# dalek-cryptography/zkp

Hardware: AMD Instinct MI355X
Metric: proofs/sec + batch-verifies/sec, CMZ13 10-attr credential, 1/2/4/8 MI355X (higher is better)
Workload: dtype u32x9 (29-bit limbs, u64 accumulate)

## Files before the change

### include/zkp_mi355x.h

```cpp
#ifndef ZKP_MI355X_H
#define ZKP_MI355X_H

#include <stddef.h>
#include <stdint.h>

#ifdef __cplusplus
extern "C" {
#endif

#define ZKP_OK 0
#define ZKP_ERR_HIP (-1)
#define ZKP_ERR_ARG (-2)
#define ZKP_ERR_NO_DEVICE (-3)
#define ZKP_ERR_OOM (-4)

#define ZKP_VARTIME 0
#define ZKP_CT 1

typedef struct zkp_ctx zkp_ctx;

int zkp_ctx_create(zkp_ctx** out, int device_id);
void zkp_ctx_destroy(zkp_ctx* ctx);
int zkp_ctx_set_stream(zkp_ctx* ctx, void* hip_stream);
int zkp_ctx_synchronize(zkp_ctx* ctx);
// ... 158 lines not shown
                  uint8_t* out );
int zkp_sc_muladd_dev(zkp_ctx* ctx, uint64_t n, const uint8_t* d_a, uint32_t a_stride, const uint8_t* d_b, uint32_t b_stride, const uint8_t* d_c,
                      uint32_t c_stride, uint8_t* d_out );
int zkp_sc_random(zkp_ctx* ctx, uint64_t n, const uint8_t key[32], uint64_t nonce, uint8_t* out );
int zkp_sc_random_dev(zkp_ctx* ctx, uint64_t n, const uint8_t key[32], uint64_t nonce, uint8_t* d_out );
int zkp_sc_hash_from_bytes_sha512(zkp_ctx* ctx, uint64_t n, const uint8_t* msgs, const uint64_t* offsets , uint8_t* out );
int zkp_sc_hash_from_bytes_sha512_dev(zkp_ctx* ctx, uint64_t n, const uint8_t* d_msgs, uint64_t msgs_len, const uint64_t* d_offsets ,
                                      uint8_t* d_out );

int zkp_transcripts_append_message(zkp_ctx* ctx, uint32_t N, int shared_initial, uint8_t* ts , const char* label,
                                   const uint8_t* msgs, const uint64_t* offsets );
int zkp_transcripts_append_message_dev(zkp_ctx* ctx, uint32_t N, int shared_initial, const uint8_t* d_ts_in, uint8_t* d_ts_out,
                                       const char* label, const uint8_t* d_msgs, uint64_t msgs_len, const uint64_t* d_offsets );
int zkp_transcripts_challenge_bytes(zkp_ctx* ctx, uint32_t N, uint8_t* ts , const char* label, uint32_t len,
                                    uint8_t* out );
int zkp_transcripts_challenge_bytes_dev(zkp_ctx* ctx, uint32_t N, uint8_t* d_ts , const char* label, uint32_t len,
                                        uint8_t* d_out );
uint32_t zkp_strobe_pos_after_append(uint32_t strobe_pos, uint64_t label_len, uint64_t msg_len);

int zkp_mul_base(zkp_ctx* ctx, uint64_t n, const uint8_t* scalars , uint8_t* out );
int zkp_mul_base_dev(zkp_ctx* ctx, uint64_t n, const uint8_t* d_scalars , uint8_t* d_out );
int zkp_mul_points(zkp_ctx* ctx, uint64_t n, const uint8_t* scalars, uint32_t s_stride, const uint8_t* points, uint32_t p_stride, int flags,
                   uint8_t* out , uint8_t* status );
int zkp_mul_points_dev(zkp_ctx* ctx, uint64_t n, const uint8_t* d_scalars, uint32_t s_stride, const uint8_t* d_points, uint32_t p_stride, int flags,
                       uint8_t* d_out , uint8_t* d_status );

#define ZKP_PT_ADD 0
#define ZKP_PT_SUB 1
int zkp_add_points(zkp_ctx* ctx, uint64_t n, const uint8_t* a, uint32_t a_stride, const uint8_t* b, uint32_t b_stride, int op,
                   uint8_t* out , uint8_t* status );
int zkp_add_points_dev(zkp_ctx* ctx, uint64_t n, const uint8_t* d_a, uint32_t a_stride, const uint8_t* d_b, uint32_t b_stride, int op,
                       uint8_t* d_out , uint8_t* d_status );
int zkp_sum_points(zkp_ctx* ctx, uint32_t n_sums, const uint32_t* off , const uint32_t* pidx ,
                   const uint8_t* neg , const uint8_t* points , uint32_t n_points,
                   uint8_t* out , uint8_t* status );
int zkp_sum_points_dev(zkp_ctx* ctx, uint32_t n_sums, const uint32_t* d_off , const uint32_t* d_pidx ,
                       const uint8_t* d_neg , const uint8_t* d_points , uint32_t n_points, uint32_t n_terms,
                       uint8_t* d_out , uint8_t* d_status );
uint32_t zkp_sum_points_group(void);

#define ZKP_DLOG_FOUND 0
#define ZKP_DLOG_INVALID 1
#define ZKP_DLOG_NOT_FOUND 2
int zkp_ctx_prepare_dlog(zkp_ctx* ctx, uint32_t baby_bits);
uint32_t zkp_dlog_baby_bits(zkp_ctx* ctx);
int zkp_dlog_base(zkp_ctx* ctx, uint64_t n, const uint8_t* points , uint32_t bits, uint64_t* out , uint8_t* status );
int zkp_dlog_base_dev(zkp_ctx* ctx, uint64_t n, const uint8_t* d_points , uint32_t bits, uint64_t* d_out , uint8_t* d_status );
uint32_t zkp_dlog_group(void);
uint32_t zkp_dlog_chunk(void);
uint32_t zkp_dlog_slice_chunks(uint64_t n);

int zkp_msm_segments(zkp_ctx* ctx, uint32_t n_msm, const uint32_t* off , const uint8_t* scalars ,
                     const uint32_t* pidx , const uint8_t* points , uint32_t n_points, int flags,
                     uint8_t* out , uint8_t* status );
int zkp_msm_segments_dev(zkp_ctx* ctx, uint32_t n_msm, const uint32_t* d_off , const uint8_t* d_scalars ,
                         const uint32_t* d_pidx , const uint8_t* d_points , uint32_t n_points,
                         uint32_t n_terms, int flags, uint8_t* d_out , uint8_t* d_status );

enum {
  ZKP_K_DECODE = 0,
  ZKP_K_TERMS = 1,
  ZKP_K_REDUCE = 2,
  ZKP_K_SORT = 3,
  ZKP_K_BUCKET = 4,
  ZKP_K_COMBINE = 5,
  ZKP_K_TRANSCRIPT = 6,
  ZKP_K_SCALARS = 7,
  ZKP_K_TABLES = 8,
  ZKP_K_COUNT = 9
};
int zkp_ctx_last_timing(zkp_ctx* ctx, float* kernel_ms , float* total_ms);
int zkp_ctx_last_kernels(zkp_ctx* ctx, int kind, char* buf, size_t cap);
int zkp_ctx_set_profiling(zkp_ctx* ctx, int enabled);

#ifdef ZKP_BUILD_TEST_HOOKS
int zkp_debug_quad_selftest(zkp_ctx* ctx, uint32_t n, const uint8_t* pairs , uint8_t* out );
int zkp_debug_row_selftest(zkp_ctx* ctx, uint32_t n, const uint8_t* pairs , uint8_t* out );
int zkp_debug_wave_cycles(zkp_ctx* ctx, uint64_t* out, uint32_t cap);
int zkp_debug_sha512(zkp_ctx* ctx, uint64_t n, const uint8_t* msgs, const uint64_t* offsets , uint8_t* out );
int zkp_debug_last_schedule(zkp_ctx* ctx, char* buf, size_t cap);
int zkp_debug_ragged_blocks(const uint8_t* transcripts, uint32_t N, uint32_t* idx, uint32_t* blocks, uint32_t cap);
int zkp_debug_fill_workspace(zkp_ctx* ctx, size_t min_bytes, uint32_t word);
size_t zkp_debug_ws_bytes(zkp_ctx* ctx);
enum { ZKP_TESTOPT_DUMMY_LAUNCHES = 1001, ZKP_TESTOPT_GENERIC_CLASSIFIER = 1002, ZKP_TESTOPT_WAVE_CYCLES = 1003, ZKP_TESTOPT_PIP_MERGE = 1004, ZKP_TESTOPT_VOUCH_REDUCED = 1005 };
#endif

#ifdef __cplusplus
}
#endif
#endif
```

### zkp_amd/csrc/fused_flows.h

```cpp
#pragma once
#include "merlin_prog.h"
#include "transcript_kernels.h"

namespace zkp {

__global__ void __launch_bounds__(256)
k_wide_reduce(uint32_t n, const uint8_t* __restrict__ wide, uint8_t* __restrict__ out) {
  const uint32_t i = blockIdx.x * blockDim.x + threadIdx.x;
  if (i >= n) return;
  sc lo, hi, r;
  load_vec<2>(lo.v, wide + 64 * (size_t)i);
  load_vec<2>(hi.v, wide + 64 * (size_t)i + 32);
  sc_from_wide(r, lo, hi);
  store_vec<2>(out + 32 * (size_t)i, r.v);
}

__global__ void __launch_bounds__(256)
k_neg_reduce(uint32_t n, const uint8_t* in, uint8_t* out) {
  const uint32_t i = blockIdx.x * blockDim.x + threadIdx.x;
  if (i >= n) return;
  sc a, r;
  load_vec<2>(a.v, in + 32 * (size_t)i);
  sc_reduce(r, a);
  sc_neg(r, r);
// ... 1091 lines not shown
  if (o.end + terms_path_ws(n_points, N * T1, N * nc, tk) > ws_bound)
    return fail(ZKP_ERR_ARG, "internal: verify_core's term path does not fit the workspace its caller sized");
  const ws_view w{static_cast<char*>(c->ws)};
  tr_bufs hb{};
  hb.src[SRC_TABLE] = d_tbl; hb.src[SRC_COMS] = w.u8(o.coms);
  hb.dst[DST_CHAL] = w.u8(o.wchal);
  HIP_TRY(hipMemsetAsync(w.base + o.failed, 0, (size_t)N * 4, c->stream));
  prof_begin(c);
  const size_t lanes = std::max<size_t>((size_t)N * T1, (size_t)N * nc) + 1;
  tk.throughput = throughput;
  if (pl.d_order) { tk.map.N = N; tk.map.nc = nc; tk.map.order = pl.d_order; }
  tk.stmt.off = w.u32(o.off); tk.stmt.pidx = w.u32(o.pidx);
  uint64_t* d_img = pl.img_bytes ? reinterpret_cast<uint64_t*>(w.base + o.img) : nullptr;
  offer_program(c, pl.a, N, hb, d_ts, nullptr, w.u32(o.failed), throughput, overlap, d_img);
  {
    hipStream_t main;
    int rc = side_begin(c, &main, overlap);
    if (rc) { c->pending_tr.offered = c->pending_tr.active = false; return rc; }
    if (late_inputs && late_early) {
      hipStream_t cur = c->stream;
      c->stream = main;
      rc = (*late_inputs)();
      c->stream = cur;
      late_inputs = nullptr;
      if (rc) { (void)side_end(c, main, overlap); c->pending_tr.offered = c->pending_tr.active = false; return rc; }
    }
    if (!stmt_classify_applies(tk, N * T1))
      hipLaunchKernelGGL(k_stmt_index, grid1(lanes, 256), dim3(256), 0, c->stream, N, T1, nc, pl.s.ns, pl.d_tarr, pl.d_tarr + nc + 1 + T1, w.u32(o.off), w.u32(o.pidx));
    rc = msm_terms_path(c, N * nc, w.u32(o.off), nullptr, w.u32(o.pidx), d_tbl, n_points, N * T1, ZKP_VARTIME, w.u8(o.coms), w.u8(o.st8), nullptr, o.end, true, PH_POINTS, tk);
    const int rc2 = side_end(c, main, overlap);
    if (rc || rc2) { c->pending_tr.offered = c->pending_tr.active = false; return rc ? rc : rc2; }
  }
  if (late_inputs) { const int rc = (*late_inputs)(); if (rc) return rc; }
  run_program_pending(c, pl.a, N, hb, d_ts, nullptr, w.u32(o.failed), throughput, d_img);
  prof_mark(c, ZKP_K_TRANSCRIPT);
  hipLaunchKernelGGL(k_neg_reduce, grid1(N, 256), dim3(256), 0, c->stream, N, d_claim, w.u8(o.mc));
  if (T1) hipLaunchKernelGGL(k_stmt_scalars, grid1((size_t)N * T1, 256), dim3(256), 0, c->stream, N, T1, m, pl.d_tarr + nc + 1, d_resp, w.u8(o.mc), w.u8(o.sc), 0u);
  prof_mark(c, ZKP_K_SCALARS);
  HIP_TRY(hipGetLastError());
  int rc = side_join(c, overlap);
  if (rc) return rc;
  rc = msm_terms_path(c, N * nc, w.u32(o.off), w.u8(o.sc), w.u32(o.pidx), d_tbl, n_points, N * T1, ZKP_VARTIME, w.u8(o.coms), w.u8(o.st8), nullptr, o.end, true, PH_SCALARS, tk);
  if (rc) return rc;
  run_program(c, pl.b, N, hb, d_ts, nullptr, w.u32(o.failed), throughput, d_img);
  prof_mark(c, ZKP_K_TRANSCRIPT);
  hipLaunchKernelGGL(k_wide_reduce, grid1(N, 256), dim3(256), 0, c->stream, N, w.u8(o.wchal), w.u8(o.chal));
  hipLaunchKernelGGL(k_verify_finish, grid1(N, 256), dim3(256), 0, c->stream, N, nc, pl.s.ns, m, w.u8(o.chal), d_claim, d_resp, w.u8(o.st8), w.u32(o.failed),
                     reinterpret_cast<const dev_affine*>(w.base + o.end), pl.d_tarr + nc + 1 + 2 * (size_t)T1, (uint32_t)pl.s.unref.size(), d_results);
  prof_mark(c, ZKP_K_SCALARS);
  HIP_TRY(hipGetLastError());
  return ZKP_OK;
}

struct batch_inter { size_t sc, failed, flags, wchal, mc, part, img, end; };
batch_inter batch_carve(const fused_plan& pl, size_t start, uint32_t K = 1) {
  const size_t N = pl.N, ns = pl.s.ns, N_each = N / (K ? K : 1), total = (size_t)K * ns + ((size_t)pl.s.ni + pl.s.nc) * N, nblk = (size_t)K * ((N_each + 255) / 256);
  carve cv;
  cv.off = start;
  batch_inter o;
  o.sc = cv.take(total * 32 + 32);
  o.failed = cv.take(N * 4 + 4);
  o.flags = cv.take((size_t)K * 4);
  o.wchal = cv.take(N * 64 + 64);
  o.mc = cv.take(N * 32 + 32);
  o.part = cv.take((ns ? ns : 1) * (nblk ? nblk : 1) * 32);
  o.img = cv.take(pl.img_bytes);
  o.end = cv.off;
  return o;
}
size_t optional_many_ws(uint64_t n_each, uint32_t K) {
  switch (pick_c(n_each)) {
    case 7: return pip_ws<7>(n_each, K);
    case 10: return pip_ws<10>(n_each, K);
    case 11: return pip_ws<11>(n_each, K);
    default: return pip_ws<16>(n_each, K);
  }
}
int batch_core(zkp_ctx* c, const fused_plan& pl, const batch_inter& o, uint8_t* d_ts, uint8_t* d_pts, const uint8_t* d_coms,
               const uint8_t* d_resp, const uint8_t* d_w, uint8_t* d_out ,
               uint32_t* d_status , bool throughput, uint32_t K = 1,
               bool overlap = false, const std::function<int()>* late_ts = nullptr, const std::function<int()>* late_scalars = nullptr, bool late_early = false) {
  const uint32_t N = pl.N, nc = pl.s.nc, ns = pl.s.ns, ni = pl.s.ni, N_each = N / K;
  const size_t n_each = (size_t)ns + ((size_t)ni + nc) * N_each;
  const ws_view w{static_cast<char*>(c->ws)};
  uint32_t* shared = nullptr;
  if (K > 1) {
    shared = w.u32(o.flags);
    HIP_TRY(hipMemsetAsync(shared, 0, (size_t)K * 4, c->stream));
  } else if (N && n_each > kSmallOptional && pl.a.n) {
    shared = w.u32(o.failed) + N;
  }
  if (!shared) HIP_TRY(hipMemsetAsync(d_status, 0, 8, c->stream));
  prof_begin(c);
  ZKP_SCHED(c, STATUS_SHARED, shared != nullptr);
  uint64_t* d_img = pl.img_bytes ? reinterpret_cast<uint64_t*>(w.base + o.img) : nullptr;
  const bool split = overlap && K == 1 && N && shared && transcript_steps(c, pl.a, N, throughput, d_img);
  if (N) {
    tr_bufs hb{};
    hb.src[SRC_TABLE] = d_pts; hb.src[SRC_COMS] = d_coms;
    hb.dst[DST_CHAL] = w.u8(o.wchal);
    if (split) {
      run_program(c, pl.a, N, hb, d_ts, nullptr, w.u32(o.failed), throughput, d_img, true, 1);
      hipStream_t main;
      int rc = side_begin(c, &main, true);
      if (rc) return rc;
      if (late_early) {
        hipStream_t cur = c->stream;
        c->stream = main;
        if (late_ts) rc = (*late_ts)();
        if (!rc && late_scalars) rc = (*late_scalars)();
        c->stream = cur;
        late_ts = late_scalars = nullptr;
        if (rc) { (void)side_end(c, main, true); return rc; }
      }
      if (nc) hipLaunchKernelGGL(k_transpose_commitments, grid1((size_t)N * nc, 256), dim3(256), 0, c->stream, N, nc, d_coms, d_pts + 32 * ((size_t)ns + (size_t)ni * N));
      rc = msm_optional_impl(c, n_each, w.u8(o.sc), d_pts, d_out, d_status, o.end, shared, 1);
      const int rc2 = side_end(c, main, true);
      if (rc || rc2) return rc ? rc : rc2;
      if (late_ts) { rc = (*late_ts)(); if (rc) return rc; }
      run_program(c, pl.a, N, hb, d_ts, nullptr, w.u32(o.failed), throughput, d_img, true, 2);
    } else {
      if (late_ts) { const int rc = (*late_ts)(); if (rc) return rc; }
      run_program(c, pl.a, N, hb, d_ts, nullptr, w.u32(o.failed), throughput, d_img, true);
    }
    prof_mark(c, ZKP_K_TRANSCRIPT);
    if (late_scalars) { const int rc = (*late_scalars)(); if (rc) return rc; }
    const size_t lanes = std::max<size_t>(std::max<size_t>(N, (size_t)N * nc), (size_t)N * pl.s.m);
    hipLaunchKernelGGL(k_batch_after_transcript, grid1(lanes, 256), dim3(256), 0, c->stream, N, N_each, nc, pl.s.m, w.u32(o.failed),
                       shared ? shared : d_status + 1, 1u, shared ? 2u : 1u, w.u8(o.wchal), w.u8(o.mc), split ? (const uint8_t*)nullptr : d_coms,
                       d_pts + 32 * ((size_t)ns + (size_t)ni * N), d_resp);
  }
  launch_coeff_build(c, pl.s, N_each, pl.d_inc, w.u8(o.mc), d_resp, d_w, w.u8(o.sc), w.u32(o.part), K);
  prof_mark(c, ZKP_K_SCALARS);
  HIP_TRY(hipGetLastError());
  if (split) {
    const int rc = side_join(c, true);
    if (rc) return rc;
    return msm_optional_impl(c, n_each, w.u8(o.sc), d_pts, d_out, d_status, o.end, shared, 2);
  }
  if (K == 1) return msm_optional_impl(c, n_each, w.u8(o.sc), d_pts, d_out, d_status, o.end, shared);
  pip_seg seg;
  seg.K = K; seg.ns = ns; seg.N_each = N_each;
  switch (pick_c(n_each)) {
    case 7: return pip_run<7>(c, (uint32_t)n_each, w.u8(o.sc), d_pts, d_out, d_status, o.end, shared, seg);
    case 10: return pip_run<10>(c, (uint32_t)n_each, w.u8(o.sc), d_pts, d_out, d_status, o.end, shared, seg);
    case 11: return pip_run<11>(c, (uint32_t)n_each, w.u8(o.sc), d_pts, d_out, d_status, o.end, shared, seg);
    default: return pip_run<16>(c, (uint32_t)n_each, w.u8(o.sc), d_pts, d_out, d_status, o.end, shared, seg);
  }
}

struct each_inter { size_t failed, wchal, mc, off, sc, pidx, out, st8, img, end; };
each_inter each_carve(const fused_plan& pl, size_t start) {
  const size_t N = pl.N, K = (size_t)pl.s.np + pl.s.nc;
  carve cv;
  cv.off = start;
  each_inter o;
  o.failed = cv.take(N * 4 + 4);
  o.wchal = cv.take(N * 64 + 64);
  o.mc = cv.take(N * 32 + 32);
  o.off = cv.take((N + 1) * 4);
  o.sc = cv.take(N * K * 32 + 32);
  o.pidx = cv.take(N * K * 4 + 4);
  o.out = cv.take(N * 32 + 32);
  o.st8 = cv.take(N + 4);
  o.img = cv.take(pl.img_bytes);
  o.end = cv.off;
  return o;
}
terms_cfg each_terms_cfg(const fused_plan& pl) {
  terms_cfg k;
  k.max_tables = pl.N >= 2 ? pl.s.ns : 0;
  k.max_ladder = (uint32_t)std::min<uint64_t>(((uint64_t)pl.s.ni + pl.s.nc) * pl.N + pl.s.ns, 0xffffffffu);
  k.teeth = pl.N >= 6 ? 16 : 4;
  return k;
}
struct straus_inter { size_t pts, tab, digits, spart, end; };
constexpr uint32_t kStrausMaxLanes = 8, kStrausMaxOpsPerLane = 60;
constexpr uint32_t kStrausWinParts = 32, kStrausWinMaxProofs = 65536;
inline uint32_t straus_win_parts(const zkp_ctx* c, const fused_plan& pl) {
  const uint32_t K = pl.s.np + pl.s.nc, N = pl.N;
  if (K > 64 || c->each_straus_lanes) return 0;
  if (c->each_straus_wins) return c->each_straus_wins;
  return N < kStrausWinMaxProofs ? kStrausWinParts : 0;
}
inline uint32_t straus_lanes(const zkp_ctx* c, const fused_plan& pl) {
  const uint32_t K = pl.s.np + pl.s.nc, N = pl.N;
  uint32_t L = c->each_straus_lanes ? std::min<uint32_t>(c->each_straus_lanes, kStrausMaxLanes) : (N >= 65536 ? 1u : (N >= 32768 ? 2u : (N >= 16384 ? 4u : 8u)));
  while (L < kStrausMaxLanes && (K + L - 1) / L > kStrausMaxOpsPerLane) L *= 2;
  return std::max(1u, std::min(std::min(L, kStrausMaxLanes), K));
}
inline bool each_uses_straus(const zkp_ctx* c, const fused_plan& pl) {
  const uint64_t K = (uint64_t)pl.s.np + pl.s.nc;
  return c->each_straus && K >= 4 && (K + kStrausMaxLanes - 1) / kStrausMaxLanes <= kStrausMaxOpsPerLane;
}
straus_inter straus_carve(const zkp_ctx* c, const fused_plan& pl, size_t start) {
  const size_t N = pl.N, K = (size_t)pl.s.np + pl.s.nc, n_points = (size_t)pl.s.ns + (size_t)pl.s.ni * N + N * pl.s.nc;
  carve cv;
  cv.off = start;
  straus_inter o;
  o.pts = cv.take(n_points * sizeof(dev_affine));
  o.tab = cv.take(n_points * 8 * sizeof(straus_entry) + 128);
  o.digits = cv.take(N * K * 9 * 4);
  o.spart = cv.take(N * (std::max(kStrausMaxLanes, straus_win_parts(c, pl)) + 1) * sizeof(dev_ext));
  o.end = cv.off;
  return o;
}
int each_core(zkp_ctx* c, const fused_plan& pl, const each_inter& o, uint8_t* d_ts, const uint8_t* d_tbl, const uint8_t* d_resp,
              const uint8_t* d_w, uint8_t* d_results, bool overlap) {
  const uint32_t N = pl.N, nc = pl.s.nc, ns = pl.s.ns, ni = pl.s.ni, K = pl.s.np + nc;
  const uint32_t n_points = ns + ni * N + N * nc;
  const ws_view w{static_cast<char*>(c->ws)};
  const uint8_t* d_coms = d_tbl + 32 * ((size_t)ns + (size_t)ni * N);
  tr_bufs hb{};
  hb.src[SRC_TABLE] = d_tbl; hb.src[SRC_COMS] = d_coms;
  hb.dst[DST_CHAL] = w.u8(o.wchal);
  HIP_TRY(hipMemsetAsync(w.base + o.failed, 0, (size_t)N * 4, c->stream));
  prof_begin(c);
  const bool straus = each_uses_straus(c, pl);
  straus_inter so{};
  dev_affine* pts = nullptr;
  straus_entry* tab = nullptr;
  if (straus) {
    so = straus_carve(c, pl, o.end);
    if (so.end > c->ws_bytes) return fail(ZKP_ERR_ARG, "internal: workspace too small");
// ... 292 lines not shown
```

### zkp_amd/csrc/zkp_kernels.hip

```cpp
#include <hip/hip_runtime.h>
#include <sys/syscall.h>
#include <unistd.h>
#include <cctype>
#include <cstdio>
#include <cstring>
#include <algorithm>
#include <atomic>
#include <functional>
#include <map>
#include <memory>
#include <mutex>
#include <set>
#include <string>
#include <vector>
#include "../../include/zkp_mi355x.h"
#include "dev_layout.h"

using namespace zkp;

__device__ __forceinline__ uint32_t sel8(const uint32_t w[8], int j) {
  uint32_t r = w[0];
#pragma unroll
  for (int i = 1; i < 8; ++i) r = (j == i) ? w[i] : r;
  return r;
}

#include "sc25519.h"
#include "hot_tables.h"
#include "quad.h"
#include "rowfe.h"
#include "comb_tables.h"
#include "point_mul.h"
#include "point_sum.h"
#include "dlog.h"
#include "transcript_kernels.h"
#include "sha512.h"

__global__ void __launch_bounds__(256, 2)
k_decode_affine(uint32_t n, const uint8_t* __restrict__ enc, dev_affine* __restrict__ out, const uint32_t* __restrict__ only) {
  const uint32_t i = blockIdx.x * blockDim.x + threadIdx.x;
  if (i >= n) return;
  if (only && !only[i]) { out[i].valid = 1; return; }
  uint32_t w[8];
  load_vec<2>(w, enc + 32 * (size_t)i);
  ge_p3 p;
  const uint32_t ok = ristretto_decode(p, w);
  store_affine(out + i, p, ok);
}

__device__ __forceinline__ void term_generic(uint32_t t, const uint8_t* __restrict__ scalars, const uint32_t* __restrict__ pidx,
                                             uint32_t n_points, const dev_affine* __restrict__ pts, dev_ext* __restrict__ partial) {
  uint32_t s[8], e[8], top;
  load_vec<2>(s, scalars + 32 * (size_t)t);
  sc_add_pattern(e, top, s, 0xAAAAAAAAu);
  ge_p3 P, P2, acc;
  const uint32_t pi = pidx[t];
  load_affine(P, pts + (pi < n_points ? pi : 0u));
  ge_cached c1, c2;
  ge_to_cached(c1, P);
  ge_double<true>(P2, P);
  ge_to_cached(c2, P2);
  ge_identity(acc);
  fe_cmov(acc.X, P.X, top);
  fe_cmov(acc.Y, P.Y, top);
  fe_cmov(acc.T, P.T, top);
#pragma unroll 1
  for (int j = 7; j >= 0; --j) {
    uint32_t cur = sel8(e, j);
#pragma unroll 1
    for (int k = 0; k < 16; ++k) {
      const uint32_t d = cur >> 30;
      cur <<= 2;
      ge_double<false>(acc, acc);
      ge_double<true>(acc, acc);
      const uint32_t neg = (uint32_t)(d < 2);
      const uint32_t mag = neg ? 2u - d : d - 2u;
      ge_cached sel;
      ge_cached_identity(sel);
      ge_cached_cmov(sel, c1, (uint32_t)(mag == 1));
      ge_cached_cmov(sel, c2, (uint32_t)(mag == 2));
      ge_cached_cneg(sel, neg);
      ge_add_cached(acc, acc, sel);
    }
  }
  store_ext(partial + t, acc);
}

__global__ void __launch_bounds__(256, 2)
k_terms_r4(uint32_t n_terms, const uint8_t* __restrict__ scalars, const uint32_t* __restrict__ pidx,
           uint32_t n_points, const dev_affine* __restrict__ pts, dev_ext* __restrict__ partial) {
  const uint32_t t = blockIdx.x * blockDim.x + threadIdx.x;
  if (t < n_terms) term_generic(t, scalars, pidx, n_points, pts, partial);
}

#ifdef ZKP_BUILD_TEST_HOOKS
__device__ uint64_t* g_wave_cycles = nullptr;
__device__ uint32_t g_wave_cycles_cap = 0;
#define ZKP_WAVE_T0 const uint64_t wave_t0_ = __builtin_readcyclecounter();
#define ZKP_WAVE_T1(cls) do { const uint64_t dt_ = __builtin_readcyclecounter() - wave_t0_; const uint32_t wi_ = blockIdx.x * 4 + (threadIdx.x >> 6); \
  if (g_wave_cycles && (threadIdx.x & 63u) == 0 && wi_ < g_wave_cycles_cap) g_wave_cycles[wi_] = ((uint64_t)(cls) << 56) | (dt_ & 0x00ffffffffffffffull); } while (0)
#else
#define ZKP_WAVE_T0
#define ZKP_WAVE_T1(cls)
#endif

enum : int { LOOKUP_XBAR = 0, LOOKUP_SCAN = 1, LOOKUP_LDS = 2 };
template <int LOOKUP>
constexpr int terms_lds_uint4() {
  if (LOOKUP == LOOKUP_XBAR) return XBAR_LDS_UINT4 > 512 ? XBAR_LDS_UINT4 : 512;
  return HOT_ROW_CHUNKS * HOT_COPIES > GROUP_LDS_UINT4 ? HOT_ROW_CHUNKS * HOT_COPIES : GROUP_LDS_UINT4;
// ... 276 lines not shown
  if (i < n_msm) {
    ge_p3 acc;
    const uint32_t g = msm_of_lane(map, i);
    const uint32_t bad = msm_sum(acc, g, off, pidx, n_points, pts, partial);
    status[g] = (STATUS_T)bad;
    ristretto_dc_state s;
    ristretto_dc_prepare(s, x, acc);
    const uint32_t zero = fe_iszero(x);
    zflag[i] = (uint8_t)zero;
    if (zero) fe_1(x);
    uint32_t* st = states + (size_t)i * 54;
#pragma unroll
    for (int k = 0; k < 9; ++k) {
      st[k] = s.e.v[k]; st[9 + k] = s.f.v[k]; st[18 + k] = s.g.v[k]; st[27 + k] = s.h.v[k]; st[36 + k] = s.eg.v[k]; st[45 + k] = s.fh.v[k];
      xs[(size_t)i * 9 + k] = x.v[k];
    }
  }
  tree_put(tree, ENC_BLOCK + tid, x);
  __syncthreads();
  tree_up(tree, tid);
  if (tid < 9) bprod[(size_t)blockIdx.x * 9 + tid] = tree.node[1][tid];
}

__global__ void __launch_bounds__(ENC_BLOCK)
k_encode_invert(uint32_t n_blocks, const uint32_t* __restrict__ bprod, uint32_t* __restrict__ binv) {
  __shared__ enc_tree tree;
  encode_invert_block(tree, threadIdx.x, blockIdx.x * ENC_BLOCK + threadIdx.x, n_blocks, bprod, binv);
}

__global__ void __launch_bounds__(ENC_BLOCK, 2)
k_encode_finish(uint32_t n_msm, const uint32_t* __restrict__ off, const uint32_t* __restrict__ pidx, uint32_t n_points,
                const dev_affine* __restrict__ pts, const dev_ext* __restrict__ partial, const uint32_t* __restrict__ states,
                const uint32_t* __restrict__ xs, const uint32_t* __restrict__ binv, const uint8_t* __restrict__ zflag,
                const uint8_t* __restrict__ status8, const uint32_t* __restrict__ status32, uint8_t* __restrict__ out, const msm_map map) {
  __shared__ enc_tree tree;
  const int tid = threadIdx.x;
  const uint32_t i = blockIdx.x * ENC_BLOCK + tid;
  fe x;
  fe_1(x);
  if (i < n_msm) {
#pragma unroll
    for (int k = 0; k < 9; ++k) x.v[k] = xs[(size_t)i * 9 + k];
    FE_TRACK(fe_set_ub_tight(x));
  }
  tree_put(tree, ENC_BLOCK + tid, x);
  __syncthreads();
  tree_up(tree, tid);
  if (tid < 9) tree.node[1][tid] = binv[(size_t)blockIdx.x * 9 + tid];
  __syncthreads();
  tree_down(tree, tid);
  if (i >= n_msm) return;
  const uint32_t g = msm_of_lane(map, i);
  uint32_t w[8];
  if (zflag[i]) {
    ge_p3 acc;
    msm_sum(acc, g, off, pidx, n_points, pts, partial);
    ge_double<true>(acc, acc);
    ristretto_encode(w, acc);
  } else {
    ristretto_dc_state s;
    const uint32_t* st = states + (size_t)i * 54;
#pragma unroll
    for (int k = 0; k < 9; ++k) {
      s.e.v[k] = st[k]; s.f.v[k] = st[9 + k]; s.g.v[k] = st[18 + k]; s.h.v[k] = st[27 + k]; s.eg.v[k] = st[36 + k]; s.fh.v[k] = st[45 + k];
    }
    fe inv;
    tree_get(inv, tree, ENC_BLOCK + tid);
    ristretto_dc_finish(w, s, inv);
  }
  const uint32_t bad = status8 ? (uint32_t)status8[g] : status32[g];
  if (bad) {
#pragma unroll
    for (int k = 0; k < 8; ++k) w[k] = 0;
  }
  store_vec<2>(out + 32 * (size_t)g, w);
}

__global__ void k_iota_single_msm(uint32_t n, uint32_t* __restrict__ pidx, uint32_t* __restrict__ off) {
  const uint32_t i = blockIdx.x * blockDim.x + threadIdx.x;
  if (i < n) pidx[i] = i;
  if (i == 0) { off[0] = 0; off[1] = n; }
}

template <int C>
struct pip_cfg {
  static constexpr int W = (256 + C - 1) / C;
  static constexpr int W1 = W + 1;
  static constexpr uint32_t B = 1u << (C - 1);
  static constexpr uint32_t B1 = B + 1;
  static constexpr uint32_t kword(int j) {
    uint32_t r = 0;
    for (int w = 0; w < W; ++w) {
      const int bit = C - 1 + C * w;
      if (bit / 32 == j) r |= 1u << (bit % 32);
    }
    return r;
  }
};

struct pip_seg {
  uint32_t K = 1, ns = 0, N_each = 0;
};
__device__ __forceinline__ void pip_seg_src(const pip_seg& seg, uint32_t b, uint32_t l, size_t& si, size_t& pi) {
  si = pi = l;
  if (seg.K > 1) {
    if (l < seg.ns) {
      si = (size_t)b * seg.ns + l;
    } else {
      const uint32_t q = l - seg.ns, r = q / seg.N_each, j = q - r * seg.N_each;
      const size_t col = ((size_t)r * seg.K + b) * seg.N_each + j;
      si = (size_t)seg.K * seg.ns + col;
      pi = (size_t)seg.ns + col;
    }
  }
}

template <int C, int PHASE = 3>
__global__ void __launch_bounds__(256, 2)
k_pip_prepare(uint32_t n, const pip_seg seg, const uint8_t* __restrict__ scalars, const uint8_t* __restrict__ points,
              dev_niels* __restrict__ niels, uint32_t* __restrict__ digits, uint32_t* __restrict__ invalid) {
  using cfg = pip_cfg<C>;
  const uint32_t i = blockIdx.x * blockDim.x + threadIdx.x, b = blockIdx.y;
  if (i >= n) return;
  size_t si, pi;
  pip_seg_src(seg, b, i, si, pi);
  niels += (size_t)b * n;
  digits += (size_t)b * cfg::W1 * n;
  if constexpr (PHASE & 1) {
    uint32_t w[8];
    load_vec<2>(w, points + 32 * pi);
    ge_p3 p;
    const uint32_t ok = ristretto_decode(p, w);
    ge_niels q;
    ge_affine_to_niels(q, p);
    store_niels(niels + i, q, ok);
    if (!ok) atomicOr(invalid + b, 1u);
  }
  if constexpr (!(PHASE & 2)) return;
  uint32_t s[8], e[10];
  load_vec<2>(s, scalars + 32 * si);
  const uint32_t flip = sc_fold_sign(s);
  {
    uint64_t c = 0;
#pragma unroll
    for (int j = 0; j < 9; ++j) {
      c += (uint64_t)(j < 8 ? s[j] : 0u) + cfg::kword(j);
      e[j] = (uint32_t)c;
      c >>= 32;
    }
    e[9] = 0;
  }
#pragma unroll
  for (int w = 0; w < cfg::W1; ++w) {
    const int pos = C * w, lo = pos >> 5, sh = pos & 31;
    uint32_t v = e[lo] >> sh;
    if (sh + C > 32) v |= e[lo + 1] << (32 - sh);
    v &= (1u << C) - 1u;
    uint32_t mag, neg;
    if (w < cfg::W) {
      neg = (uint32_t)(v < cfg::B);
      mag = neg ? cfg::B - v : v - cfg::B;
    } else {
      neg = 0;
      mag = v;
    }
    digits[(size_t)w * n + i] = mag | ((neg ^ flip) << 31);
  }
}

__device__ __forceinline__ uint32_t part_len(uint32_t cnt, uint32_t L) {
  const uint32_t r = (uint32_t)ceilf(sqrtf((float)cnt));
  return r > 4 * L ? 4 * L : (r > L ? r : L);
}
__device__ __forceinline__ uint32_t part_count(uint32_t cnt, uint32_t L) {
  const uint32_t pl = part_len(cnt, L);
  return (cnt + pl - 1) / pl;
}

__global__ void __launch_bounds__(256)
k_pip_scan(uint32_t bins, uint32_t L, const uint32_t* __restrict__ hist, uint32_t* __restrict__ start,
           uint32_t* __restrict__ cursor, uint32_t* __restrict__ vstart) {
  __shared__ uint32_t part[256];
  __shared__ uint32_t vpart[256];
  const uint32_t w = blockIdx.x, tid = threadIdx.x;
  const uint32_t chunk = (bins + 255) / 256;
  const uint32_t lo = min(tid * chunk, bins), hi = min(lo + chunk, bins);
  const uint32_t* h = hist + (size_t)w * bins;
  uint32_t sum = 0, vsum = 0;
  for (uint32_t b = lo; b < hi; ++b) { sum += h[b]; vsum += part_count(h[b], L); }
  part[tid] = sum;
  vpart[tid] = vsum;
  __syncthreads();
  for (uint32_t d = 1; d < 256; d <<= 1) {
    const uint32_t v = tid >= d ? part[tid - d] : 0;
    const uint32_t vv = tid >= d ? vpart[tid - d] : 0;
    __syncthreads();
    part[tid] += v;
    vpart[tid] += vv;
    __syncthreads();
  }
  uint32_t run = part[tid] - sum, vrun = vpart[tid] - vsum;
  for (uint32_t b = lo; b < hi; ++b) {
    start[(size_t)w * bins + b] = run;
    cursor[(size_t)w * bins + b] = run;
    vstart[(size_t)w * (bins + 1) + b] = vrun;
    run += h[b];
    vrun += part_count(h[b], L);
  }
  if (tid == 255) vstart[(size_t)w * (bins + 1) + bins] = vpart[255];
}

template <int C>
struct sort_cfg {
  static constexpr int THREADS = C >= 16 ? 1024 : 256;
  static constexpr uint32_t TILE = C >= 16 ? 65536u : 2048u;
};

template <int C>
__global__ void __launch_bounds__(sort_cfg<C>::THREADS)
k_pip_tile_hist(uint32_t n, const uint32_t* __restrict__ digits, uint32_t* __restrict__ tilehist) {
  using cfg = pip_cfg<C>;
  __shared__ uint32_t h[cfg::B1];
  const uint32_t w = blockIdx.y, t = blockIdx.x, tiles = gridDim.x;
  for (uint32_t b = threadIdx.x; b < cfg::B1; b += blockDim.x) h[b] = 0;
  __syncthreads();
  const uint32_t lo = t * sort_cfg<C>::TILE, hi = min(n, lo + sort_cfg<C>::TILE);
  const uint32_t* d = digits + (size_t)w * n;
  for (uint32_t i = lo + threadIdx.x; i < hi; i += blockDim.x) {
    const uint32_t mag = d[i] & 0x7fffffffu;
    if (mag) atomicAdd(&h[mag], 1u);
  }
  __syncthreads();
  uint32_t* out = tilehist + ((size_t)w * tiles + t) * cfg::B1;
  for (uint32_t b = threadIdx.x; b < cfg::B1; b += blockDim.x) out[b] = h[b];
}

__global__ void __launch_bounds__(256)
k_pip_tile_total(uint32_t bins, uint32_t tiles, uint32_t total, const uint32_t* __restrict__ tilehist, uint32_t* __restrict__ hist) {
  const uint32_t g = blockIdx.x * blockDim.x + threadIdx.x;
  if (g >= total) return;
  const uint32_t w = g / bins, b = g - w * bins;
  const uint32_t* p = tilehist + (size_t)w * tiles * bins + b;
  uint32_t sum = 0, t = 0;
  for (; t + 8 <= tiles; t += 8) {
    uint32_t v[8];
#pragma unroll
    for (int k = 0; k < 8; ++k) v[k] = p[(size_t)(t + k) * bins];
#pragma unroll
    for (int k = 0; k < 8; ++k) sum += v[k];
  }
  for (; t < tiles; ++t) sum += p[(size_t)t * bins];
  hist[g] = sum;
}
__global__ void __launch_bounds__(256)
k_pip_tile_base(uint32_t bins, uint32_t tiles, uint32_t total, const uint32_t* __restrict__ start, uint32_t* __restrict__ tilehist) {
  const uint32_t g = blockIdx.x * blockDim.x + threadIdx.x;
  if (g >= total) return;
  const uint32_t w = g / bins, b = g - w * bins;
  uint32_t* p = tilehist + (size_t)w * tiles * bins + b;
  uint32_t run = start[g], t = 0;
  for (; t + 8 <= tiles; t += 8) {
    uint32_t v[8];
#pragma unroll
    for (int k = 0; k < 8; ++k) v[k] = p[(size_t)(t + k) * bins];
#pragma unroll
    for (int k = 0; k < 8; ++k) { p[(size_t)(t + k) * bins] = run; run += v[k]; }
  }
  for (; t < tiles; ++t) {
    const uint32_t c = p[(size_t)t * bins];
    p[(size_t)t * bins] = run;
    run += c;
  }
}

template <int C>
__global__ void __launch_bounds__(sort_cfg<C>::THREADS)
k_pip_tile_scatter(uint32_t n, const uint32_t* __restrict__ digits, const uint32_t* __restrict__ tilehist,
                   uint32_t* __restrict__ sorted) {
  using cfg = pip_cfg<C>;
  __shared__ uint32_t base[cfg::B1];
  const uint32_t tiles = gridDim.x, WK = gridDim.y, lin = blockIdx.x + blockIdx.y * tiles, full = (WK & ~7u) * tiles;
  uint32_t w, t;
#ifdef ZKP_AB_PLAIN_SCATTER
  if (false) {
#else
  if (lin < full) {
#endif
    const uint32_t grp = lin / (8u * tiles), r = lin - grp * 8u * tiles;
    w = grp * 8u + (r & 7u);
    t = r >> 3;
  } else {
    w = blockIdx.y;
    t = blockIdx.x;
  }
  const uint32_t* in = tilehist + ((size_t)w * tiles + t) * cfg::B1;
  for (uint32_t b = threadIdx.x; b < cfg::B1; b += blockDim.x) base[b] = in[b];
  __syncthreads();
  const uint32_t lo = t * sort_cfg<C>::TILE, hi = min(n, lo + sort_cfg<C>::TILE);
  const uint32_t* d = digits + (size_t)w * n;
  uint32_t* out = sorted + (size_t)w * n;
  for (uint32_t i = lo + threadIdx.x; i < hi; i += blockDim.x) {
    const uint32_t key = d[i], mag = key & 0x7fffffffu;
    if (mag) out[atomicAdd(&base[mag], 1u)] = i | (key & 0x80000000u);
  }
}

__global__ void __launch_bounds__(256)
k_pip_vmap(uint32_t bins, uint32_t total, uint32_t vmax, const uint32_t* __restrict__ vstart, uint32_t* __restrict__ vmap) {
  const uint32_t g = blockIdx.x * blockDim.x + threadIdx.x;
  uint32_t w = 0, b = 0, v0 = 0, v1 = 0;
  if (g < total) {
    w = g / bins; b = g - w * bins;
    const uint32_t* vs = vstart + (size_t)w * (bins + 1);
    v0 = vs[b]; v1 = vs[b + 1];
  }
  uint64_t bigmask = __ballot(v1 - v0 > 64u);
  while (bigmask) {
    const int src = __ffsll((unsigned long long)bigmask) - 1;
    bigmask &= bigmask - 1;
    const uint32_t bw = (uint32_t)__shfl((int)w, src), bb = (uint32_t)__shfl((int)b, src), b0 = (uint32_t)__shfl((int)v0, src), b1 = (uint32_t)__shfl((int)v1, src);
    for (uint32_t v = b0 + (threadIdx.x & 63u); v < b1; v += 64) vmap[(size_t)bw * vmax + v] = bb;
  }
  if (v1 - v0 <= 64u)
    for (uint32_t v = v0; v < v1; ++v) vmap[(size_t)w * vmax + v] = b;
}

__global__ void __launch_bounds__(256, 2)
k_pip_bucket_part(uint32_t n, uint32_t W1, uint32_t bins, uint32_t L, uint32_t vmax, const uint32_t* __restrict__ start,
                  const uint32_t* __restrict__ hist, const uint32_t* __restrict__ vstart, const uint32_t* __restrict__ vmap,
                  const uint32_t* __restrict__ sorted, const dev_niels* __restrict__ niels,
                  dev_ext* __restrict__ parts) {
  const uint32_t v = blockIdx.x * blockDim.x + threadIdx.x;
  const uint32_t w = blockIdx.y;
  const uint32_t* vs = vstart + (size_t)w * (bins + 1);
  if (v >= vs[bins]) return;
  const uint32_t b = vmap[(size_t)w * vmax + v], g = w * bins + b;
  const uint32_t pl = part_len(hist[g], L);
  const uint32_t first = (v - vs[b]) * pl;
  const uint32_t cnt = min(pl, hist[g] - first);
  const uint32_t* lst = sorted + (size_t)w * n + start[g] + first;
  niels += (size_t)(w / W1) * n;
  ge_p3 acc;
  ge_niels qa, qb;
  uint32_t ia = lst[0], ib = 0;
  load_niels(qa, niels + (ia & 0x7fffffffu));
  if (1 < cnt) { ib = lst[1]; load_niels(qb, niels + (ib & 0x7fffffffu)); }
  ge_niels_cneg(qa, ia >> 31);
  ge_from_niels(acc, qa);
#pragma unroll 1
  for (uint32_t k = 1; k < cnt; k += 2) {
    if (k + 1 < cnt) { ia = lst[k + 1]; load_niels(qa, niels + (ia & 0x7fffffffu)); }
    ge_niels_cneg(qb, ib >> 31);
    ge_madd(acc, acc, qb);
    if (k + 1 < cnt) {
      if (k + 2 < cnt) { ib = lst[k + 2]; load_niels(qb, niels + (ib & 0x7fffffffu)); }
      ge_niels_cneg(qa, ia >> 31);
      ge_madd(acc, acc, qa);
    }
  }
  store_ext(parts + (size_t)w * vmax + v, acc);
}

constexpr uint32_t kMergeSeqParts = 128;
template <bool LANE>
__global__ void __launch_bounds__(256, 2)
k_pip_bucket_merge(uint32_t bins, uint32_t total, uint32_t vmax, const uint32_t* __restrict__ vstart,
                   const dev_ext* __restrict__ parts, dev_ext* __restrict__ buckets) {
  __shared__ uint32_t big[LANE ? 256 : 64];
  __shared__ uint32_t n_big;
  __shared__ uint32_t red[64][4][9];
  const uint32_t gt = blockIdx.x * blockDim.x + threadIdx.x;
  const uint32_t g = LANE ? gt : gt >> 2, qi = threadIdx.x >> 2;
  const int q = (int)(threadIdx.x & 3u);
  if (threadIdx.x == 0) n_big = 0;
  __syncthreads();
  if (g < total) {
    const uint32_t w = g / bins, b = g - w * bins;
    const uint32_t* vs = vstart + (size_t)w * (bins + 1);
    const uint32_t v0 = vs[b], v1 = vs[b + 1];
    const dev_ext* p = parts + (size_t)w * vmax;
    if (v1 - v0 > kMergeSeqParts) {
// ... 33 lines not shown
  }
  __syncthreads();
  const uint32_t nb = n_big;
#pragma unroll 1
  for (uint32_t i = 0; i < nb; ++i) {
    const uint32_t gb = big[i], w = gb / bins, b = gb - w * bins;
    const uint32_t* vs = vstart + (size_t)w * (bins + 1);
    const uint32_t v0 = vs[b], v1 = vs[b + 1];
    const dev_ext* p = parts + (size_t)w * vmax;
    qpt acc;
    q_identity(acc, q);
    if (v0 + qi < v1) q_load_ext(acc, p + v0 + qi, q);
#pragma unroll 1
    for (uint32_t v = v0 + qi + 64; v < v1; v += 64) {
      qpt t;
      q_load_ext(t, p + v, q);
      q_add(acc, acc, t, q);
    }
#pragma unroll
    for (int k = 0; k < 9; ++k) red[qi][q][k] = acc.c.v[k];
    __syncthreads();
#pragma unroll 1
    for (uint32_t d = 32; d >= 1; d >>= 1) {
      if (qi < d) {
        qpt t;
#pragma unroll
        for (int k = 0; k < 9; ++k) t.c.v[k] = red[qi + d][q][k];
        q_add(acc, acc, t, q);
#pragma unroll
        for (int k = 0; k < 9; ++k) red[qi][q][k] = acc.c.v[k];
      }
      __syncthreads();
    }
    if (qi == 0) q_store_ext(buckets + gb, acc, q);
    __syncthreads();
  }
}

__device__ __forceinline__ void pip_reduce_quad(uint32_t g, int q, uint32_t n_out, uint32_t in_stride, uint32_t out_stride, int level, int m, int shift,
                                                const dev_ext* __restrict__ A_in, const dev_ext* __restrict__ R_in,
                                                dev_ext* __restrict__ A_out, dev_ext* __restrict__ R_out) {
  const uint32_t w = g / n_out, j = g - w * n_out;
  const dev_ext* rin = R_in + (size_t)w * in_stride + (size_t)m * j;
  qpt run, U, t;
  q_identity(run, q);
  q_identity(U, q);
  if (level == 0 && j == n_out - 1) {
    q_load_ext(run, rin + m, q);
    U = run;
  }
#pragma unroll 1
  for (int i = m - 1; i >= 1; --i) {
    q_load_ext(t, rin + i, q);
    q_add(run, run, t, q);
    q_add(U, U, run, q);
  }
  q_load_ext(t, rin, q);
  q_add(run, run, t, q);
#pragma unroll 1
  for (int k = 0; k < shift; ++k) q_double(U, U, q);
  if (level > 0) {
    const dev_ext* ain = A_in + (size_t)w * in_stride + (size_t)m * j;
#pragma unroll 1
    for (int i = 0; i < m; ++i) {
      q_load_ext(t, ain + i, q);
      q_add(U, U, t, q);
    }
  }
  q_store_ext(A_out + (size_t)w * out_stride + j, U, q);
  if (R_out) q_store_ext(R_out + (size_t)w * out_stride + j, run, q);
}
__global__ void __launch_bounds__(256, 2)
k_pip_reduce_lvl(uint32_t n_out, uint32_t total, uint32_t in_stride, uint32_t out_stride, int level, int m, int shift,
                 const dev_ext* __restrict__ A_in, const dev_ext* __restrict__ R_in,
                 dev_ext* __restrict__ A_out, dev_ext* __restrict__ R_out) {
  const uint32_t gt = blockIdx.x * blockDim.x + threadIdx.x;
  const uint32_t g = gt >> 2;
  const int q = (int)(gt & 3u);
  if (g >= total) return;
  pip_reduce_quad(g, q, n_out, in_stride, out_stride, level, m, shift, A_in, R_in, A_out, R_out);
}

__global__ void __launch_bounds__(256)
k_pip_combine(int W1, int C, uint32_t in_stride, int level, int m, int shift, const dev_ext* __restrict__ A_in, const dev_ext* __restrict__ R_in,
              dev_ext* __restrict__ T_all, const uint32_t* __restrict__ invalid, uint8_t* __restrict__ out_point, uint32_t* __restrict__ status,
              uint32_t shared_flags ) {
  const uint32_t b = blockIdx.x;
  dev_ext* T = T_all + (size_t)b * W1;
  const uint32_t g = threadIdx.x >> 2;
  const int q = (int)(threadIdx.x & 3u);
  if (g < (uint32_t)W1) pip_reduce_quad(b * (uint32_t)W1 + g, q, 1u, in_stride, 1u, level, m, shift, A_in, R_in, T_all, nullptr);
  __syncthreads();
  __shared__ uint32_t Tl[64 * 36];
  if (g < (uint32_t)W1) {
    qpt t;
    q_load_ext(t, T + g, q);
    if (g + 1 < (uint32_t)W1) {
      qcached cc;
      q_to_cached(cc, t, q);
      t.c = cc.c;
    }
#pragma unroll
    for (int i = 0; i < 9; ++i) Tl[36 * g + 9 * q + i] = t.c.v[i];
  }
  __syncthreads();
  if (threadIdx.x < 64) {
    rowctx rc;
    row_init(rc);
    const uint32_t at = 9u * rc.r + (rc.live ? rc.k : 0u);
    uint32_t acc = rc.live ? Tl[36 * (W1 - 1) + at] : 0u;
#pragma unroll 1
    for (int k = W1 - 2; k >= 0; --k) {
#pragma unroll 1
      for (int d = 0; d < C; ++d) acc = row_double(rc, acc);
      const uint32_t t = rc.live ? Tl[36 * k + at] : 0u;
      acc = row_add_cached(rc, acc, t);
    }
    if (rc.live) Tl[at] = acc;
  }
  __syncthreads();
  if (threadIdx.x >= 4) return;
  qpt acc;
#pragma unroll
  for (int i = 0; i < 9; ++i) acc.c.v[i] = Tl[9 * q + i];
  ge_p3 full;
  q_gather(full, acc);
  uint32_t o[8];
  if (shared_flags) {
#pragma unroll
    for (int k = 0; k < 8; ++k) o[k] = 0;
    o[0] = (fe_iszero(full.X) | fe_iszero(full.Y)) ^ 1u;
  } else {
    ristretto_encode(o, full);
  }
  if (q != 0) return;
  const uint32_t flags = invalid[b];
  const uint32_t bad = flags & 1u;
  if (bad) {
#pragma unroll
    for (int k = 0; k < 8; ++k) o[k] = 0;
  }
  store_vec<2>(out_point + 32 * (size_t)b, o);
  if (shared_flags) { status[2 * b] = bad; status[2 * b + 1] = (flags >> 1) & 1u; }
  else status[b] = bad;
}

#ifdef ZKP_BUILD_TEST_HOOKS
__global__ void __launch_bounds__(256, 2)
k_debug_quad(uint32_t n, const uint8_t* __restrict__ enc, uint8_t* __restrict__ out) {
  const uint32_t gt = blockIdx.x * blockDim.x + threadIdx.x;
  const uint32_t i = gt >> 2;
  const int q = (int)(gt & 3u);
  if (i >= n) return;
  uint32_t w[8];
  ge_p3 P, Q, R;
  load_vec<2>(w, enc + 64 * (size_t)i);
  ristretto_decode(P, w);
  load_vec<2>(w, enc + 64 * (size_t)i + 32);
  ristretto_decode(Q, w);
  qpt p, s, r;
  p.c = q == 0 ? P.X : (q == 1 ? P.Y : (q == 2 ? P.Z : P.T));
  s.c = q == 0 ? Q.X : (q == 1 ? Q.Y : (q == 2 ? Q.Z : Q.T));
  __shared__ dev_niels nl[64];
  ge_niels qn;
  ge_affine_to_niels(qn, Q);
  if (q == 0) store_niels(&nl[threadIdx.x >> 2], qn, 1u);
  __syncthreads();
  uint32_t o[8];
  for (int op = 0; op < 4; ++op) {
    if (op == 0) q_double(r, p, q);
    else if (op == 1) q_add(r, p, s, q);
    else { qcached c; q_load_niels(c, &nl[threadIdx.x >> 2], q, op == 3 ? 1u : 0u); q_add_cached(r, p, c, q); }
    q_gather(R, r);
    ristretto_encode(o, R);
    if (q == 0) store_vec<2>(out + 128 * (size_t)i + 32 * op, o);
  }
}
__global__ void __launch_bounds__(64)
k_debug_row(uint32_t n, const uint8_t* __restrict__ enc, uint8_t* __restrict__ out) {
  const uint32_t i = blockIdx.x;
  if (i >= n) return;
  __shared__ uint32_t S[3 * 36];
  if (threadIdx.x == 0) {
    uint32_t w[8];
    ge_p3 P, Q;
    load_vec<2>(w, enc + 64 * (size_t)i);
    ristretto_decode(P, w);
    load_vec<2>(w, enc + 64 * (size_t)i + 32);
    ristretto_decode(Q, w);
    fe c[4], d2;
    fe_sub(c[0], Q.Y, Q.X);
    fe_carry(c[0], c[0]);
    fe_add(c[1], Q.Y, Q.X);
    fe_carry(c[1], c[1]);
    fe_add(c[2], Q.Z, Q.Z);
// ... 524 lines not shown
  {
    uint32_t s[8];
    dlog_small_scalar(s, live ? j0 << (baby_bits - 1u) : 0ull);
    ge_p3 A, H;
    dlog_mul_base(A, s, table);
    ge_identity(H);
    if (live) load_ext(H, halves + p);
    ge_cached ca;
    ge_to_cached(ca, A);
    ge_sub_cached(P, H, ca);
  }
#pragma unroll 1
  for (uint32_t t = 0; t < steps; ++t) {
    uint32_t w[8];
    dlog_group_encode(w, P, tree, tid);
    if (live) {
      const uint32_t i = dlog_probe(w, slots, rows, baby_bits);
      const uint64_t k = ((j0 + t) << baby_bits) + i;
      if (i != DLOG_NONE && dlog_in_range(k, bits)) {
        out[p] = k;
        status[p] = (uint8_t)ZKP_DLOG_FOUND;
        live = 0;
      }
    }
    if (__syncthreads_or((int)live) == 0) break;
    ge_cached st;
    dlog_load_cached(st, consts + 36);
    ge_sub_cached(P, P, st);
  }
}

static thread_local std::string g_last_error = "";
struct zkp_ctx;
static std::mutex g_ctx_mu;
static std::set<zkp_ctx*> g_live_ctx;
static std::atomic<uint64_t> g_ctx_next_id{1};

static int fail(int code, const std::string& msg) {
  g_last_error = msg;
  return code;
}
#define HIP_TRY(expr)                                                                          \
  do {                                                                                         \
    hipError_t e_ = (expr);                                                                    \
    if (e_ != hipSuccess)                                                                      \
      return fail(e_ == hipErrorOutOfMemory ? ZKP_ERR_OOM : ZKP_ERR_HIP,                       \
                  std::string(#expr) + ": " + hipGetErrorString(e_));                          \
  } while (0)

constexpr int kMaxEvents = 32;
struct zkp_ctx {
  uint64_t uid = 0;
  int device = 0;
  hipStream_t own_stream = nullptr;
  hipStream_t stream = nullptr;
  hipStream_t side_stream = nullptr;
  hipEvent_t ev_fork = nullptr, ev_join = nullptr;
  bool prof_suspended = false;
  bool capturing = false;
  uint64_t batch_encode_min = 65536;
  bool batch_encode_user = false;
  int comb_teeth = 4;
  int ct_single_use_tables = -1;
  struct { bool offered = false, active = false; const tr_op* ops = nullptr; uint32_t n_ops = 0; const uint64_t* tables = nullptr; uint32_t N = 0; tr_bufs bufs{};
           uint8_t* ts = nullptr; uint32_t* saved = nullptr; uint32_t* failed = nullptr; uint32_t tail = 0;
           bool steps = false; tr_steps_dev sd; uint64_t* img = nullptr; } pending_tr;
  int debug_dummy_launches = 0;
  bool stmt_classify = true;
  int fuse_tables_transcript = -1;
  int tables_lane = -1;
  int comb_split = -1;
  int grouped_comb = -1;
  int ladder_interleave = -1;
  static constexpr uint32_t kInterleaveLadderBlocks = 256;
  bool each_straus = true;
  uint32_t each_straus_lanes = 0;
  uint32_t each_straus_wins = 0;
  int ct_lookup = 0;
#ifdef ZKP_BUILD_TEST_HOOKS
  uint64_t* wave_cycles = nullptr;
  static constexpr uint32_t kWaveCyclesCap = 1u << 20;
  enum { SCH_BATCH_ENCODE, SCH_ENC_GROUPS, SCH_OPT_PIP, SCH_PIP_C, SCH_PIP_PART, SCH_STATUS_SHARED, SCH_LAT_SPLIT, SCH_GROUPED, SCH_COMB_MIN,
         SCH_LADDER_INTERLEAVE, SCH_RIDERS, SCH_STRAUS_LANES, SCH_STRAUS_WINS, SCH_TR_LANES, SCH_TR_STEPS, SCH_FUSE_TT, SCH_TERMS_SPLIT,
         SCH_RAGGED_CLASSES, SCH_RAGGED_COMPILED, SCH_RAGGED_BASE, SCH_FUSED_PLANS, SCH_PIP_MERGE, SCH_PIP_BUCKETS, SCH_NO_CARRY, SCH_SIGN_FOLD, SCH_COUNT };
  int64_t sched[SCH_COUNT] = {-1, -1, -1, -1, -1, -1, -1, -1, -1, -1, -1, -1, -1, -1, -1, -1, -1, -1, -1, -1, -1, -1, -1, -1, -1};
  int debug_pip_merge = 0;
  bool debug_vouch_reduced = false;
#endif
  static constexpr size_t kGroupedCombTerms = 400000;
  static constexpr size_t kSplitCombTerms = 8192;
  bool dev_overlap = false;
  bool dev_latency = false;
  bool rider_tables = true;
  bool joint_ladder = true;
  bool tr_steps = true;
  int tr_lanes = -1;
  static constexpr size_t kWideCallTerms = 250000, kWideCallProofs = 8192;
  static constexpr size_t kVeryWideCallProofs = 65536;
  uint32_t ct_comb_min(bool throughput, size_t n_terms) const {
    return ct_single_use_tables < 0 ? (throughput && n_terms >= kWideCallTerms ? 2u : 1u) : (ct_single_use_tables ? 1u : 2u);
  }
  void* ws = nullptr;
  size_t ws_bytes = 0;
  uint64_t ws_generation = 0, plans_generation = 0;
  bool profiling = false;
  hipEvent_t ev[kMaxEvents] = {};
  int ev_kind[kMaxEvents] = {};
  int n_ev = 0;
  float kernel_ms[ZKP_K_COUNT] = {};
  float total_ms = 0;
  std::string kernel_names[ZKP_K_COUNT];
  dev_niels* hot_tables = nullptr;
  uint32_t* hot_reg_words = nullptr;
  int32_t* hot_reg_slot = nullptr;
  char* hot_scratch = nullptr;
  std::string hot_key[HOT_SLOTS];
  uint64_t hot_used[HOT_SLOTS] = {};
  uint64_t hot_tick = 0;
  uint32_t hot_nreg = 0;
  dev_niels* base_table = nullptr;
  uint32_t dlog_baby_bits = 0;
  uint32_t* dlog_rows = nullptr;
  dlog_slot* dlog_slots = nullptr;
  uint32_t* dlog_consts = nullptr;
  std::map<std::string, void*> fused_plans;
  std::map<std::string, void*> ragged_progs, ragged_bases;
  uint64_t ragged_tick = 0;
  struct job_t {
    char kind = 0;
    hipEvent_t done = nullptr;
    uint8_t* pin = nullptr;
    size_t pin_bytes = 0;
    uint32_t K = 0;
    int* verdicts = nullptr;
    int* invalid_point = nullptr;
    uint8_t* results = nullptr;
    size_t n_results = 0;
    hipError_t copy_err = hipSuccess;
    hipEvent_t tev[4] = {};
    bool timed = false;
    float ms[3] = {};
    struct out_copy { void* dst; const void* src; size_t bytes; };
    std::vector<out_copy> outs;
    hipEvent_t copied = nullptr;
    bool copies_issued = false;
    bool inline_out = false;
  } job;
  int defer_d2h = -1;
  bool sync_throughput = false;
  size_t ws_limit = 0;
  bool hot_registry_uploaded = false;
};
void free_fused_plans(zkp_ctx* c);
static void free_dlog_table(zkp_ctx* c) {
  if (c->dlog_rows) (void)hipFree(c->dlog_rows);
  if (c->dlog_slots) (void)hipFree(c->dlog_slots);
  if (c->dlog_consts) (void)hipFree(c->dlog_consts);
  c->dlog_rows = nullptr;
  c->dlog_slots = nullptr;
  c->dlog_consts = nullptr;
  c->dlog_baby_bits = 0;
}
void free_ragged_progs(zkp_ctx* c);

namespace {

struct carve {
  size_t off = 0;
// ... 264 lines not shown
      ZKP_SCHED(c, SIGN_FOLD, (no_carry && lookup == LOOKUP_XBAR) ? 1 : 0);
#define ZKP_LAUNCH_TERMS(CT_, TEETH_, LK_) launch_terms_split<CT_, TEETH_, LK_>(c, grid, k.max_ladder != 0, d_scalars, d_pidx, n_points, comb, slot_of, class_start, blk_start, list, pts, ladder, k.max_ladder, part, comb_split ? 1u : 0u, pair_on ? k.stmt.pair : (const uint32_t*)nullptr, k.stmt.T, no_carry)
      if (lookup == LOOKUP_XBAR) {
        if (flags == ZKP_CT) { if (k.teeth == 16) ZKP_LAUNCH_TERMS(true, 16, LOOKUP_XBAR); else ZKP_LAUNCH_TERMS(true, 4, LOOKUP_XBAR); }
        else { if (k.teeth == 16) ZKP_LAUNCH_TERMS(false, 16, LOOKUP_XBAR); else ZKP_LAUNCH_TERMS(false, 4, LOOKUP_XBAR); }
      }
#if ZKP_HOT_W <= 6
      else if (lookup == LOOKUP_SCAN) {
        if (k.teeth == 16) ZKP_LAUNCH_TERMS(true, 16, LOOKUP_SCAN); else ZKP_LAUNCH_TERMS(true, 4, LOOKUP_SCAN);
      } else {
        if (flags == ZKP_CT) { if (k.teeth == 16) ZKP_LAUNCH_TERMS(true, 16, LOOKUP_LDS); else ZKP_LAUNCH_TERMS(true, 4, LOOKUP_LDS); }
        else { if (k.teeth == 16) ZKP_LAUNCH_TERMS(false, 16, LOOKUP_LDS); else ZKP_LAUNCH_TERMS(false, 4, LOOKUP_LDS); }
      }
#endif
#undef ZKP_LAUNCH_TERMS
    }
  } else {
    if (n_points && (phase & PH_POINTS)) hipLaunchKernelGGL(k_decode_affine, grid1(n_points, 256), dim3(256), 0, c->stream, n_points, d_points, pts, (const uint32_t*)nullptr);
    prof_mark(c, ZKP_K_DECODE);
    if (n_terms && (phase & PH_SCALARS)) hipLaunchKernelGGL(k_terms_r4, grid1(n_terms, 256), dim3(256), 0, c->stream, n_terms, d_scalars, d_pidx, n_points, pts, part);
  }
  if (!(phase & PH_SCALARS)) { HIP_TRY(hipGetLastError()); return ZKP_OK; }
  prof_mark(c, ZKP_K_TERMS);
  if (k.terms_only) { HIP_TRY(hipGetLastError()); return ZKP_OK; }
  if (n_msm && batched_encode) {
    uint32_t* states = reinterpret_cast<uint32_t*>(base + o.states);
    uint32_t* xs = reinterpret_cast<uint32_t*>(base + o.xs);
    uint32_t* bprod = reinterpret_cast<uint32_t*>(base + o.bprod);
    uint32_t* binv = bprod + (size_t)enc_blocks * 9;
    uint8_t* zflag = reinterpret_cast<uint8_t*>(base + o.zflag);
    if (d_status8)
      hipLaunchKernelGGL(k_encode_prepare<uint8_t>, dim3(enc_blocks), dim3(ENC_BLOCK), 0, c->stream, n_msm, d_off, d_pidx, n_points, pts, part, states, xs, bprod, zflag, d_status8, k.map);
    else
      hipLaunchKernelGGL(k_encode_prepare<uint32_t>, dim3(enc_blocks), dim3(ENC_BLOCK), 0, c->stream, n_msm, d_off, d_pidx, n_points, pts, part, states, xs, bprod, zflag, d_status32, k.map);
    hipLaunchKernelGGL(k_encode_invert, dim3(enc_groups), dim3(ENC_BLOCK), 0, c->stream, enc_blocks, bprod, binv);
    hipLaunchKernelGGL(k_encode_finish, dim3(enc_blocks), dim3(ENC_BLOCK), 0, c->stream, n_msm, d_off, d_pidx, n_points, pts, part, states, xs, binv, zflag,
                       (const uint8_t*)d_status8, (const uint32_t*)d_status32, d_out, k.map);
    prof_note(c, ZKP_K_REDUCE, "k_encode_prepare;k_encode_invert;k_encode_finish");
  } else if (n_msm) {
    if (d_status8)
      hipLaunchKernelGGL(k_reduce_encode<uint8_t>, grid1(n_msm, 256), dim3(256), 0, c->stream, n_msm, d_off, d_pidx, n_points, pts, part, d_out, d_status8, k.map);
    else
      hipLaunchKernelGGL(k_reduce_encode<uint32_t>, grid1(n_msm, 256), dim3(256), 0, c->stream, n_msm, d_off, d_pidx, n_points, pts, part, d_out, d_status32, k.map);
    prof_note(c, ZKP_K_REDUCE, "k_reduce_encode");
  }
  prof_mark(c, ZKP_K_REDUCE);
  HIP_TRY(hipGetLastError());
  return ZKP_OK;
}

inline uint32_t pip_part_len(uint64_t n) { return n < (1u << 18) ? 16u : (n < (1u << 21) ? 32u : 64u); }
template <int C>
size_t pip_vmax(uint64_t n) { return (size_t)(n / pip_part_len(n)) + pip_cfg<C>::B1 + 1; }

template <int C>
uint32_t pip_tiles(uint64_t n) { return (uint32_t)((n + sort_cfg<C>::TILE - 1) / sort_cfg<C>::TILE); }

template <int C>
size_t pip_ws(uint64_t n, uint32_t K = 1) {
  using cfg = pip_cfg<C>;
  const size_t WK = (size_t)cfg::W1 * K;
  carve cv;
  cv.take((size_t)K * n * sizeof(dev_niels));
  cv.take(WK * n * 4);
  cv.take(WK * n * 4);
  cv.take(WK * cfg::B1 * 4 * 3);
  cv.take(WK * (cfg::B1 + 1) * 4);
  cv.take(WK * pip_tiles<C>(n) * cfg::B1 * 4);
  cv.take(WK * pip_vmax<C>(n) * sizeof(dev_ext));
  cv.take(WK * pip_vmax<C>(n) * 4);
  cv.take((size_t)K * 4 + 256);
  cv.take(WK * cfg::B1 * sizeof(dev_ext));
  cv.take(WK * (cfg::B + 8) * sizeof(dev_ext) * 2);
  return cv.off;
}

template <int C>
int pip_run(zkp_ctx* c, uint32_t n, const uint8_t* d_scalars, const uint8_t* d_points, uint8_t* d_out,
            uint32_t* d_status, size_t ws_reserved, uint32_t* shared_flags, const pip_seg seg = pip_seg(), int phases = 3) {
  using cfg = pip_cfg<C>;
  const uint32_t K = seg.K;
  const size_t WK = (size_t)cfg::W1 * K;
  if (WK > 65535) return fail(ZKP_ERR_ARG, "too many batches in one call");
  carve cv;
  cv.off = ws_reserved;
  char* base = static_cast<char*>(c->ws);
  dev_niels* niels = reinterpret_cast<dev_niels*>(base + cv.take((size_t)K * n * sizeof(dev_niels)));
  uint32_t* digits = reinterpret_cast<uint32_t*>(base + cv.take(WK * n * 4));
  uint32_t* sorted = reinterpret_cast<uint32_t*>(base + cv.take(WK * n * 4));
  const size_t nb = WK * cfg::B1;
  if (nb * 4 > 0xffffffffull) return fail(ZKP_ERR_ARG, "too many batches in one call");
  uint32_t* hist = reinterpret_cast<uint32_t*>(base + cv.take(nb * 4 * 3));
  uint32_t* start = hist + nb;
  uint32_t* cursor = start + nb;
  uint32_t* vstart = reinterpret_cast<uint32_t*>(base + cv.take(WK * (cfg::B1 + 1) * 4));
  const uint32_t tiles = pip_tiles<C>(n);
  uint32_t* tilehist = reinterpret_cast<uint32_t*>(base + cv.take(WK * tiles * cfg::B1 * 4));
  const uint32_t L = pip_part_len(n);
  const size_t vmax = pip_vmax<C>(n);
  ZKP_SCHED(c, PIP_C, C);
  ZKP_SCHED(c, PIP_PART, L);
  dev_ext* parts = reinterpret_cast<dev_ext*>(base + cv.take(WK * vmax * sizeof(dev_ext)));
  uint32_t* vmap = reinterpret_cast<uint32_t*>(base + cv.take(WK * vmax * 4));
  uint32_t* invalid = reinterpret_cast<uint32_t*>(base + cv.take((size_t)K * 4 + 256));
  if (shared_flags) invalid = shared_flags;
  dev_ext* buckets = reinterpret_cast<dev_ext*>(base + cv.take(nb * sizeof(dev_ext)));
  const size_t lvl_cap = WK * (cfg::B + 8);
  dev_ext* lvlA = reinterpret_cast<dev_ext*>(base + cv.take(lvl_cap * sizeof(dev_ext) * 2));
  dev_ext* lvlR = lvlA + lvl_cap;
  if (cv.off > c->ws_bytes) return fail(ZKP_ERR_ARG, "internal: workspace too small");

  if (phases == 1) {
    if (!shared_flags) return fail(ZKP_ERR_ARG, "internal: split prepare without the caller's flag words");
    hipLaunchKernelGGL((k_pip_prepare<C, 1>), dim3((n + 255) / 256, K), dim3(256), 0, c->stream, n, seg, d_scalars, d_points, niels, digits, invalid);
    HIP_TRY(hipGetLastError());
    return ZKP_OK;
  }
  if (!shared_flags) HIP_TRY(hipMemsetAsync(invalid, 0, (size_t)K * 4, c->stream));
  prof_note(c, ZKP_K_DECODE, "k_pip_prepare<" + std::to_string(C) + ">");
  if (phases == 2) hipLaunchKernelGGL((k_pip_prepare<C, 2>), dim3((n + 255) / 256, K), dim3(256), 0, c->stream, n, seg, d_scalars, d_points, niels, digits, invalid);
  else hipLaunchKernelGGL((k_pip_prepare<C, 3>), dim3((n + 255) / 256, K), dim3(256), 0, c->stream, n, seg, d_scalars, d_points, niels, digits, invalid);
  prof_mark(c, ZKP_K_DECODE);
  hipLaunchKernelGGL(k_pip_tile_hist<C>, dim3(tiles, (unsigned)WK), dim3(sort_cfg<C>::THREADS), 0, c->stream, n, digits, tilehist);
  hipLaunchKernelGGL(k_pip_tile_total, grid1(nb, 256), dim3(256), 0, c->stream, cfg::B1, tiles, (uint32_t)nb, tilehist, hist);
  hipLaunchKernelGGL(k_pip_scan, dim3((unsigned)WK), dim3(256), 0, c->stream, cfg::B1, L, hist, start, cursor, vstart);
  hipLaunchKernelGGL(k_pip_tile_base, grid1(nb, 256), dim3(256), 0, c->stream, cfg::B1, tiles, (uint32_t)nb, start, tilehist);
  hipLaunchKernelGGL(k_pip_tile_scatter<C>, dim3(tiles, (unsigned)WK), dim3(sort_cfg<C>::THREADS), 0, c->stream, n, digits, tilehist, sorted);
  prof_mark(c, ZKP_K_SORT);
  hipLaunchKernelGGL(k_pip_vmap, grid1(nb, 256), dim3(256), 0, c->stream, cfg::B1, (uint32_t)nb, (uint32_t)vmax, vstart, vmap);
  hipLaunchKernelGGL(k_pip_bucket_part, dim3((unsigned)((vmax + 255) / 256), (unsigned)WK), dim3(256), 0, c->stream, n, (uint32_t)cfg::W1, cfg::B1, L, (uint32_t)vmax,
                     start, hist, vstart, vmap, sorted, niels, parts);
  constexpr size_t MERGE_LANE_MIN_BUCKETS = (size_t)1 << 19;
#ifdef ZKP_BUILD_TEST_HOOKS
  const bool lane_merge = c->debug_pip_merge ? c->debug_pip_merge == 2 : nb >= MERGE_LANE_MIN_BUCKETS;
#else
  const bool lane_merge = nb >= MERGE_LANE_MIN_BUCKETS;
#endif
  ZKP_SCHED(c, PIP_MERGE, lane_merge ? 1 : 0);
  ZKP_SCHED(c, PIP_BUCKETS, nb);
  if (lane_merge) hipLaunchKernelGGL(k_pip_bucket_merge<true>, grid1(nb, 256), dim3(256), 0, c->stream, cfg::B1, (uint32_t)nb, (uint32_t)vmax, vstart, parts, buckets);
  else hipLaunchKernelGGL(k_pip_bucket_merge<false>, grid1(nb * 4, 256), dim3(256), 0, c->stream, cfg::B1, (uint32_t)nb, (uint32_t)vmax, vstart, parts, buckets);
  prof_mark(c, ZKP_K_BUCKET);
  const dev_ext* Ain = nullptr;
  const dev_ext* Rin = buckets;
  uint32_t in_stride = cfg::B1, n_in = cfg::B;
  size_t lvl_off = 0;
  int level = 0;
  int shift = 0;
  static_assert(cfg::W1 <= 64, "k_pip_combine runs the last tree level with one quad per window in one 256-lane block");
  while (n_in > 1) {
    int lg = 0;
    while ((1u << lg) < n_in) ++lg;
    const int mbits = (level == 0 && lg % 3) ? lg % 3 : 3;
    const uint32_t m = 1u << mbits, n_out = n_in >> mbits;
    dev_ext* Aout = lvlA + lvl_off;
    dev_ext* Rout = lvlR + lvl_off;
    const uint32_t total = (uint32_t)WK * n_out;
    if (n_out == 1) {
      hipLaunchKernelGGL(k_pip_combine, dim3(K), dim3(256), 0, c->stream, cfg::W1, C, in_stride, level, (int)m, shift, Ain, Rin, Aout, invalid, d_out, d_status, shared_flags ? 1u : 0u);
      break;
    }
    hipLaunchKernelGGL(k_pip_reduce_lvl, grid1((size_t)total * 4, 256), dim3(256), 0, c->stream, n_out, total, in_stride, n_out, level, (int)m, shift,
                       Ain, Rin, Aout, Rout);
    Ain = Aout;
    Rin = Rout;
    in_stride = n_out;
    n_in = n_out;
    lvl_off += total;
    shift += mbits;
    ++level;
  }
  prof_mark(c, ZKP_K_COMBINE);
  HIP_TRY(hipGetLastError());
  return ZKP_OK;
}

int pick_c(uint64_t n) {
  if (n < (1u << 12)) return 7;
  if (n < (1u << 13)) return 10;
  if (n < (1u << 21)) return 11;
  return 16;
}
constexpr uint64_t kSmallOptional = 192;

terms_cfg host_terms_cfg(const zkp_ctx* c, uint32_t n_terms, const uint32_t* pidx, const uint8_t* points, uint32_t n_points, uint32_t comb_min) {
  std::vector<uint32_t> uses(n_points, 0);
  for (uint32_t t = 0; t < n_terms; ++t) ++uses[pidx[t]];
  std::vector<std::pair<uint64_t, int>> hot;
  for (int sl = 0; sl < HOT_SLOTS; ++sl)
    if (!c->hot_key[sl].empty()) { uint64_t w; memcpy(&w, c->hot_key[sl].data(), 8); hot.emplace_back(w, sl); }
  std::sort(hot.begin(), hot.end());
  std::vector<char> is_hot(n_points, 0);
  bool shared = false;
  for (uint32_t p = 0; p < n_points; ++p) {
    if (!uses[p] || hot.empty()) continue;
    uint64_t w;
    memcpy(&w, points + 32 * (size_t)p, 8);
    for (auto it = std::lower_bound(hot.begin(), hot.end(), std::make_pair(w, -1)); it != hot.end() && it->first == w; ++it)
      if (memcmp(c->hot_key[it->second].data(), points + 32 * (size_t)p, 32) == 0) { is_hot[p] = 1; break; }
  }
  for (uint32_t p = 0; p < n_points; ++p) shared |= !is_hot[p] && uses[p] >= 2;
  if (comb_min == 1 && !shared) comb_min = 2;
  uint64_t n_tab = 0, n_lad = 0, tab_terms = 0;
  for (uint32_t p = 0; p < n_points; ++p) {
    if (!uses[p] || is_hot[p]) continue;
    if (uses[p] >= comb_min) { ++n_tab; tab_terms += uses[p]; } else ++n_lad;
  }
  terms_cfg k;
  k.comb_min = comb_min;
  k.max_tables = (uint32_t)n_tab;
  k.max_ladder = (uint32_t)n_lad;
  k.teeth = pick_teeth(n_tab, tab_terms);
  return k;
}

int launch_from_uniform(zkp_ctx* c, uint64_t n, const uint8_t* d_in, uint8_t* d_out) {
  constexpr uint64_t kMaxBlocks = 2048;
  const unsigned blocks = (unsigned)std::min<uint64_t>(kMaxBlocks, (n + 255) / 256);
  hipLaunchKernelGGL(k_from_uniform, dim3(blocks), dim3(256), 0, c->stream, (uint32_t)n, d_in, d_out);
  prof_mark(c, ZKP_K_DECODE);
  HIP_TRY(hipGetLastError());
  return ZKP_OK;
}

int launch_sha512(zkp_ctx* c, uint64_t n, const uint8_t* d_msgs, uint64_t msgs_len, const uint64_t* d_offsets, uint8_t* d_out) {
  constexpr uint64_t kMaxBlocks = 2048;
  const unsigned blocks = (unsigned)std::min<uint64_t>(kMaxBlocks, (n + 255) / 256);
  hipLaunchKernelGGL(k_sha512_csr, dim3(blocks), dim3(256), 0, c->stream, (uint32_t)n, d_msgs, msgs_len, d_offsets, d_out);
  prof_mark(c, ZKP_K_TRANSCRIPT);
  HIP_TRY(hipGetLastError());
  return ZKP_OK;
}

inline unsigned sc_blocks(uint64_t n) {
  constexpr uint64_t kMaxBlocks = 2048;
  return (unsigned)std::min<uint64_t>(kMaxBlocks, (n + 255) / 256);
}
int launch_sc_invert(zkp_ctx* c, uint64_t n, const uint8_t* d_in, uint8_t* d_out) {
  hipLaunchKernelGGL(k_sc_invert, dim3(sc_blocks(n)), dim3(256), 0, c->stream, (uint32_t)n, d_in, d_out);
  prof_mark(c, ZKP_K_SCALARS);
  HIP_TRY(hipGetLastError());
  return ZKP_OK;
// ... 356 lines not shown
}

extern "C" {

const char* zkp_last_error(void) { return g_last_error.c_str(); }
#ifdef ZKP_BUILD_TEST_HOOKS
#define ZKP_VERSION_TEXT_(w) "zkp-mi355x 0.5 gfx950 (9x29-bit limbs, v_mad_u64_u32; " #w "-bit fixed-base windows)"
#define ZKP_VERSION_TEXT(w) ZKP_VERSION_TEXT_(w)
const char* zkp_version(void) { return ZKP_VERSION_TEXT(ZKP_HOT_W) " +test-hooks"; }
#else
#define ZKP_VERSION_TEXT_(w) "zkp-mi355x 0.5 gfx950 (9x29-bit limbs, v_mad_u64_u32; " #w "-bit fixed-base windows)"
#define ZKP_VERSION_TEXT(w) ZKP_VERSION_TEXT_(w)
const char* zkp_version(void) { return ZKP_VERSION_TEXT(ZKP_HOT_W); }
#endif

int zkp_ctx_create(zkp_ctx** out, int device_id) {
  if (!out) return fail(ZKP_ERR_ARG, "zkp_ctx_create: out is NULL");
  *out = nullptr;
  int count = 0;
  if (hipGetDeviceCount(&count) != hipSuccess || count == 0) return fail(ZKP_ERR_NO_DEVICE, "no HIP device visible");
  if (device_id < 0 || device_id >= count) return fail(ZKP_ERR_ARG, "device_id out of range");
  HIP_TRY(hipSetDevice(device_id));
  hipDeviceProp_t prop;
  HIP_TRY(hipGetDeviceProperties(&prop, device_id));
  if (std::string(prop.gcnArchName).rfind("gfx950", 0) != 0)
    return fail(ZKP_ERR_NO_DEVICE, std::string("device is ") + prop.gcnArchName + ", this library is built for gfx950 only");
  zkp_ctx* c = new zkp_ctx();
  c->uid = g_ctx_next_id.fetch_add(1);
  c->device = device_id;
  if (hipStreamCreateWithFlags(&c->own_stream, hipStreamNonBlocking) != hipSuccess) { delete c; return fail(ZKP_ERR_HIP, "hipStreamCreate failed"); }
  c->stream = c->own_stream;
  for (auto& e : c->ev)
    if (hipEventCreate(&e) != hipSuccess) { delete c; return fail(ZKP_ERR_HIP, "hipEventCreate failed"); }
  { std::lock_guard<std::mutex> lk(g_ctx_mu); g_live_ctx.insert(c); }
  *out = c;
  return ZKP_OK;
}

void zkp_ctx_destroy(zkp_ctx* c) {
  if (!c) return;
  { std::lock_guard<std::mutex> lk(g_ctx_mu); g_live_ctx.erase(c); }
  hipSetDevice(c->device);
  if (c->capturing) { hipGraph_t g = nullptr; hipStreamEndCapture(c->stream, &g); if (g) hipGraphDestroy(g); c->capturing = false; }
  hipStreamSynchronize(c->stream);
  if (c->job.done) hipEventDestroy(c->job.done);
  if (c->job.copied) hipEventDestroy(c->job.copied);
  for (auto& e : c->job.tev) if (e) hipEventDestroy(e);
  if (c->job.pin) hipHostFree(c->job.pin);
  if (c->ws) hipFree(c->ws);
  if (c->hot_tables) hipFree(c->hot_tables);
  if (c->base_table) hipFree(c->base_table);
  free_dlog_table(c);
  if (c->hot_reg_words) hipFree(c->hot_reg_words);
  if (c->hot_reg_slot) hipFree(c->hot_reg_slot);
  if (c->hot_scratch) hipFree(c->hot_scratch);
#ifdef ZKP_BUILD_TEST_HOOKS
  if (c->wave_cycles) { uint64_t* z = nullptr; (void)hipMemcpyToSymbol(HIP_SYMBOL(g_wave_cycles), &z, sizeof(z)); hipFree(c->wave_cycles); }
#endif
  free_fused_plans(c);
  free_ragged_progs(c);
  if (c->side_stream) hipStreamDestroy(c->side_stream);
  if (c->ev_fork) hipEventDestroy(c->ev_fork);
  if (c->ev_join) hipEventDestroy(c->ev_join);
  for (auto& e : c->ev) if (e) hipEventDestroy(e);
  if (c->own_stream) hipStreamDestroy(c->own_stream);
  delete c;
}

int zkp_ctx_set_stream(zkp_ctx* c, void* s) {
  if (!c) return fail(ZKP_ERR_ARG, "ctx is NULL");
  c->stream = s ? static_cast<hipStream_t>(s) : c->own_stream;
  return ZKP_OK;
}
int zkp_ctx_set_option(zkp_ctx* c, int option, uint64_t value) {
  if (!c) return fail(ZKP_ERR_ARG, "ctx is NULL");
  switch (option) {
    case ZKP_OPT_BATCH_ENCODE_MIN: c->batch_encode_min = value; c->batch_encode_user = true; return ZKP_OK;
    case ZKP_OPT_CT_SINGLE_USE_TABLES: c->ct_single_use_tables = value == ~0ull ? -1 : (value ? 1 : 0); return ZKP_OK;
    case ZKP_OPT_DEV_OVERLAP: c->dev_overlap = value != 0 && value != ~0ull; c->dev_latency = value == 2; return ZKP_OK;
#ifdef ZKP_BUILD_TEST_HOOKS
    case ZKP_TESTOPT_GENERIC_CLASSIFIER: c->stmt_classify = value == 0; return ZKP_OK;
    case ZKP_TESTOPT_PIP_MERGE: c->debug_pip_merge = value <= 2 ? (int)value : 0; return ZKP_OK;
    case ZKP_TESTOPT_VOUCH_REDUCED: c->debug_vouch_reduced = value != 0; return ZKP_OK;
    case ZKP_TESTOPT_DUMMY_LAUNCHES: c->debug_dummy_launches = (int)std::min<uint64_t>(value, 1000); return ZKP_OK;
    case ZKP_TESTOPT_WAVE_CYCLES: {
      HIP_TRY(hipSetDevice(c->device));
      HIP_TRY(hipStreamSynchronize(c->stream));
      uint64_t* p = nullptr;
      uint32_t cap = 0;
      if (value) {
        if (!c->wave_cycles) HIP_TRY(hipMalloc(&c->wave_cycles, sizeof(uint64_t) * zkp_ctx::kWaveCyclesCap));
        HIP_TRY(hipMemset(c->wave_cycles, 0, sizeof(uint64_t) * zkp_ctx::kWaveCyclesCap));
        p = c->wave_cycles;
        cap = zkp_ctx::kWaveCyclesCap;
      }
      HIP_TRY(hipMemcpyToSymbol(HIP_SYMBOL(g_wave_cycles), &p, sizeof(p)));
      HIP_TRY(hipMemcpyToSymbol(HIP_SYMBOL(g_wave_cycles_cap), &cap, sizeof(cap)));
      return ZKP_OK;
    }
#endif
    case ZKP_OPT_FUSE_TABLES_TRANSCRIPT: c->fuse_tables_transcript = value == ~0ull ? -1 : (value ? 1 : 0); return ZKP_OK;
    case ZKP_OPT_TABLES_LANE: c->tables_lane = value == ~0ull ? -1 : (value ? 1 : 0); return ZKP_OK;
    case ZKP_OPT_GROUPED_COMB: c->grouped_comb = value == ~0ull ? -1 : (value ? 1 : 0); return ZKP_OK;
    case ZKP_OPT_JOINT_LADDER: c->joint_ladder = value != 0; c->rider_tables = value != 2; return ZKP_OK;
    case ZKP_OPT_COMB_SPLIT: c->comb_split = value == ~0ull ? -1 : (value ? 1 : 0); return ZKP_OK;
    case ZKP_OPT_CT_LOOKUP:
      if (value == ~0ull) value = 0;
      if (value > 2 || (value && !HOT_LDS_ROWS)) return fail(ZKP_ERR_ARG, "ZKP_OPT_CT_LOOKUP: 0 (lane crossbar), 1 (masked scans), 2 (LDS rows); 1 and 2 exist for 6-bit fixed-base windows only");
      c->ct_lookup = (int)value; return ZKP_OK;
    case ZKP_OPT_LADDER_INTERLEAVE: c->ladder_interleave = value == ~0ull ? -1 : value != 0; return ZKP_OK;
    case ZKP_OPT_JOB_DEFER_D2H: c->defer_d2h = value == ~0ull ? -1 : (value ? 1 : 0); return ZKP_OK;
    case ZKP_OPT_SYNC_SCHEDULE: c->sync_throughput = value != 0 && value != ~0ull; return ZKP_OK;
    case ZKP_OPT_WS_LIMIT_BYTES: c->ws_limit = value == ~0ull ? 0 : (size_t)value; return ZKP_OK;
    case ZKP_OPT_EACH_STRAUS:
    {
      const bool wins = value > 0x200 && value <= 0x200 + 64 && ((value - 0x200) & (value - 0x201)) == 0;
      if (value != ~0ull && value > 8 && !wins)
        return fail(ZKP_ERR_ARG, "ZKP_OPT_EACH_STRAUS: 0 (off), 1 .. 8 lanes per proof, 0x200 + (1, 2, 4 .. 64) window parts per proof, or UINT64_MAX (default)");
      c->each_straus = value != 0;
      c->each_straus_lanes = (value == ~0ull || value == 0 || value > 8) ? 0u : (uint32_t)value;
      c->each_straus_wins = wins ? (uint32_t)(value - 0x200) : 0u;
      return ZKP_OK;
    }
    case ZKP_OPT_TRANSCRIPT_STEPS: c->tr_steps = value != 0; return ZKP_OK;
    case ZKP_OPT_TRANSCRIPT_LANES:
      if (value != ~0ull && value != 1 && value != 2) return fail(ZKP_ERR_ARG, "ZKP_OPT_TRANSCRIPT_LANES: 1, 2 or UINT64_MAX");
      c->tr_lanes = value == ~0ull ? -1 : (int)value;
      return ZKP_OK;
    case ZKP_OPT_COMB_TEETH:
      if (value != 4 && value != 16) return fail(ZKP_ERR_ARG, "ZKP_OPT_COMB_TEETH must be 4 or 16");
      c->comb_teeth = (int)value;
      return ZKP_OK;
    default: return fail(ZKP_ERR_ARG, "unknown option");
  }
}
int zkp_ctx_synchronize(zkp_ctx* c) {
  if (!c) return fail(ZKP_ERR_ARG, "ctx is NULL");
  HIP_TRY(hipStreamSynchronize(c->stream));
  return ZKP_OK;
}
int zkp_ctx_set_profiling(zkp_ctx* c, int enabled) {
  if (!c) return fail(ZKP_ERR_ARG, "ctx is NULL");
  c->profiling = enabled != 0;
  return ZKP_OK;
}
struct zkp_graph {
  hipGraph_t graph = nullptr;
  hipGraphExec_t exec = nullptr;
  int device = 0;
  zkp_ctx* ctx = nullptr;
  uint64_t ctx_uid = 0;
  uint64_t ws_generation = 0, plans_generation = 0;
};

int zkp_ctx_capture_begin(zkp_ctx* c) {
  if (!c) return fail(ZKP_ERR_ARG, "ctx is NULL");
  if (c->capturing) return fail(ZKP_ERR_ARG, "capture already in progress");
  HIP_TRY(hipSetDevice(c->device));
  HIP_TRY(hipStreamBeginCapture(c->stream, hipStreamCaptureModeThreadLocal));
  c->capturing = true;
  return ZKP_OK;
}
int zkp_ctx_capture_end(zkp_ctx* c, zkp_graph** out) {
  if (!c || !out) return fail(ZKP_ERR_ARG, "NULL pointer");
  *out = nullptr;
  if (!c->capturing) return fail(ZKP_ERR_ARG, "no capture in progress");
// ... 238 lines not shown
  if (!c) return fail(ZKP_ERR_ARG, "ctx is NULL");
  if (flags != ZKP_CT && flags != ZKP_VARTIME) return fail(ZKP_ERR_ARG, "flags must be ZKP_CT or ZKP_VARTIME");
  if (n_msm == 0) return ZKP_OK;
  if (!d_off || !d_out || !d_status) return fail(ZKP_ERR_ARG, "NULL device pointer");
  if (n_terms && (!d_scalars || !d_points || n_points == 0)) return fail(ZKP_ERR_ARG, "terms without scalars/points");
  if (!d_pidx && n_points != n_terms) return fail(ZKP_ERR_ARG, "without pidx, n_points must equal the number of terms");
  if (!aligned16(d_scalars) || !aligned16(d_points) || !aligned16(d_out)) return fail(ZKP_ERR_ARG, "device buffers must be 16-byte aligned");
  HIP_TRY(hipSetDevice(c->device));
  terms_cfg k;
  k.teeth = c->comb_teeth;
  k.throughput = true;
  k.comb_min = flags == ZKP_CT ? c->ct_comb_min(true, n_terms) : 2u;
  k.terms_only = true;
  carve cv;
  const size_t o_iota = cv.take(d_pidx ? 0 : (size_t)n_terms * 4);
  const segments_ws w = msm_segments_ws(n_points, n_terms, n_msm, k, cv.off);
  const int rc = ensure_ws(c, w.sum.total);
  if (rc) return rc;
  prof_begin(c);
  if (!d_pidx && n_terms) {
    uint32_t* iota = reinterpret_cast<uint32_t*>(static_cast<char*>(c->ws) + o_iota);
    hipLaunchKernelGGL(k_iota, grid1(n_terms, 256), dim3(256), 0, c->stream, n_terms, iota);
    d_pidx = iota;
  }
  return launch_msm_segments(c, n_msm, d_off, d_scalars, d_pidx, d_points, n_points, n_terms, flags, k, w, d_out, d_status);
}

int zkp_msm_segments(zkp_ctx* c, uint32_t n_msm, const uint32_t* off, const uint8_t* scalars, const uint32_t* pidx, const uint8_t* points, uint32_t n_points,
                     int flags, uint8_t* out, uint8_t* status) {
  if (!c) return fail(ZKP_ERR_ARG, "ctx is NULL");
  if (flags != ZKP_CT && flags != ZKP_VARTIME) return fail(ZKP_ERR_ARG, "flags must be ZKP_CT or ZKP_VARTIME");
  if (n_msm == 0) return ZKP_OK;
  if (!off || !out || !status) return fail(ZKP_ERR_ARG, "NULL pointer");
  if (off[0] != 0) return fail(ZKP_ERR_ARG, "off[0] must be 0");
  for (uint32_t i = 0; i < n_msm; ++i)
    if (off[i + 1] < off[i]) return fail(ZKP_ERR_ARG, "off must be non-decreasing");
  const uint32_t n_terms = off[n_msm];
  if (n_terms && (!scalars || !points || n_points == 0)) return fail(ZKP_ERR_ARG, "terms without scalars/points");
  if (!pidx && n_points != n_terms) return fail(ZKP_ERR_ARG, "without pidx, n_points must equal the number of terms");
  if (pidx)
    for (uint32_t t = 0; t < n_terms; ++t)
      if (pidx[t] >= n_points) return fail(ZKP_ERR_ARG, "pidx out of range");
  HIP_TRY(hipSetDevice(c->device));
  std::vector<uint32_t> iota;
  if (!pidx && n_terms >= 1024) {
    iota.resize(n_terms);
    for (uint32_t t = 0; t < n_terms; ++t) iota[t] = t;
  }
  terms_cfg k = n_terms >= 1024 ? host_terms_cfg(c, n_terms, pidx ? pidx : iota.data(), points, n_points, flags == ZKP_CT ? c->ct_comb_min(false, n_terms) : 2u) : terms_cfg();
#ifdef ZKP_BUILD_TEST_HOOKS
  if (c->debug_vouch_reduced && flags == ZKP_CT) k.canonical = true;
#endif
  k.terms_only = true;
  carve cv;
  const size_t o_off = cv.take((size_t)(n_msm + 1) * 4);
  const size_t o_sc = cv.take((size_t)n_terms * 32);
  const size_t o_pidx = cv.take((size_t)n_terms * 4);
  const size_t o_pts = cv.take((size_t)n_points * 32);
  const size_t o_out = cv.take((size_t)n_msm * 32);
  const size_t o_st = cv.take((size_t)n_msm);
  const segments_ws w = msm_segments_ws(n_points, n_terms, n_msm, k, cv.off);
  int rc = ensure_ws(c, w.sum.total);
  if (rc) return rc;
  char* base = static_cast<char*>(c->ws);
  HIP_TRY(hipMemcpyAsync(base + o_off, off, (size_t)(n_msm + 1) * 4, hipMemcpyHostToDevice, c->stream));
  if (n_terms) {
    HIP_TRY(hipMemcpyAsync(base + o_sc, scalars, (size_t)n_terms * 32, hipMemcpyHostToDevice, c->stream));
    if (pidx) HIP_TRY(hipMemcpyAsync(base + o_pidx, pidx, (size_t)n_terms * 4, hipMemcpyHostToDevice, c->stream));
    HIP_TRY(hipMemcpyAsync(base + o_pts, points, (size_t)n_points * 32, hipMemcpyHostToDevice, c->stream));
  }
  prof_begin(c);
  if (!pidx && n_terms) hipLaunchKernelGGL(k_iota, grid1(n_terms, 256), dim3(256), 0, c->stream, n_terms, reinterpret_cast<uint32_t*>(base + o_pidx));
  rc = launch_msm_segments(c, n_msm, reinterpret_cast<uint32_t*>(base + o_off), reinterpret_cast<uint8_t*>(base + o_sc), reinterpret_cast<uint32_t*>(base + o_pidx),
                           reinterpret_cast<uint8_t*>(base + o_pts), n_points, n_terms, flags, k, w, reinterpret_cast<uint8_t*>(base + o_out),
                           reinterpret_cast<uint8_t*>(base + o_st));
  if (rc) return rc;
  HIP_TRY(hipMemcpyAsync(out, base + o_out, (size_t)n_msm * 32, hipMemcpyDeviceToHost, c->stream));
  HIP_TRY(hipMemcpyAsync(status, base + o_st, (size_t)n_msm, hipMemcpyDeviceToHost, c->stream));
  HIP_TRY(hipStreamSynchronize(c->stream));
  return ZKP_OK;
}

static int msm_optional_impl(zkp_ctx* c, uint64_t n, const uint8_t* d_scalars, const uint8_t* d_points,
                             uint8_t* d_out, uint32_t* d_status, size_t reserved, uint32_t* shared_flags = nullptr, int phases = 3) {
  ZKP_SCHED(c, OPT_PIP, n > kSmallOptional);
  if (n <= kSmallOptional) {
    if (shared_flags) return fail(ZKP_ERR_ARG, "internal: shared flags with a small MSM");
    carve cv;
    cv.off = reserved;
    const size_t o_pidx = cv.take((size_t)(n + 1) * 4);
    const size_t o_off = cv.take(256);
    const size_t inner = cv.off;
    int rc = ensure_ws(c, inner + terms_path_ws((uint32_t)n, (uint32_t)n, 1));
    if (rc) return rc;
    char* base = static_cast<char*>(c->ws);
    uint32_t* pidx = reinterpret_cast<uint32_t*>(base + o_pidx);
    uint32_t* off = reinterpret_cast<uint32_t*>(base + o_off);
    hipLaunchKernelGGL(k_iota_single_msm, grid1(n + 1, 256), dim3(256), 0, c->stream, (uint32_t)n, pidx, off);
    return msm_terms_path(c, 1, off, d_scalars, pidx, d_points, (uint32_t)n, (uint32_t)n, ZKP_VARTIME, d_out, nullptr, d_status, inner);
  }
  if (n > 0x7fffffffull) return fail(ZKP_ERR_ARG, "n too large (max 2^31-1 terms per call)");
  const int cbits = pick_c(n);
  size_t need = 0;
  switch (cbits) {
    case 7: need = pip_ws<7>(n); break;
    case 10: need = pip_ws<10>(n); break;
    case 11: need = pip_ws<11>(n); break;
    default: need = pip_ws<16>(n); break;
  }
  int rc = ensure_ws(c, reserved + need);
  if (rc) return rc;
  switch (cbits) {
    case 7: return pip_run<7>(c, (uint32_t)n, d_scalars, d_points, d_out, d_status, reserved, shared_flags, pip_seg(), phases);
    case 10: return pip_run<10>(c, (uint32_t)n, d_scalars, d_points, d_out, d_status, reserved, shared_flags, pip_seg(), phases);
    case 11: return pip_run<11>(c, (uint32_t)n, d_scalars, d_points, d_out, d_status, reserved, shared_flags, pip_seg(), phases);
    default: return pip_run<16>(c, (uint32_t)n, d_scalars, d_points, d_out, d_status, reserved, shared_flags, pip_seg(), phases);
  }
}

int zkp_msm_optional_dev(zkp_ctx* c, uint64_t n, const uint8_t* d_scalars, const uint8_t* d_points,
                         uint8_t* d_out_point, uint32_t* d_status) {
  if (!c) return fail(ZKP_ERR_ARG, "ctx is NULL");
  if (!d_out_point || !d_status) return fail(ZKP_ERR_ARG, "NULL output pointer");
  if (n && (!d_scalars || !d_points)) return fail(ZKP_ERR_ARG, "NULL input pointer");
  if (!aligned16(d_scalars) || !aligned16(d_points) || !aligned16(d_out_point)) return fail(ZKP_ERR_ARG, "device buffers must be 16-byte aligned");
  HIP_TRY(hipSetDevice(c->device));
  prof_begin(c);
  return msm_optional_impl(c, n, d_scalars, d_points, d_out_point, d_status, 0);
}

int zkp_msm_optional(zkp_ctx* c, uint64_t n, const uint8_t* scalars, const uint8_t* points, uint8_t out_point[32], int* status) {
  if (!c) return fail(ZKP_ERR_ARG, "ctx is NULL");
  if (!out_point || !status) return fail(ZKP_ERR_ARG, "NULL output pointer");
  if (n && (!scalars || !points)) return fail(ZKP_ERR_ARG, "NULL input pointer");
  HIP_TRY(hipSetDevice(c->device));
  carve cv;
  const size_t o_sc = cv.take((size_t)n * 32 + 32);
  const size_t o_pts = cv.take((size_t)n * 32 + 32);
  const size_t o_out = cv.take(32);
  const size_t o_st = cv.take(4);
  const size_t reserved = cv.off;
  size_t need = 0;
  if (n <= kSmallOptional) {
    need = 1024 + (n + 1) * 4 + terms_path_ws((uint32_t)n, (uint32_t)n, 1);
  } else {
    switch (pick_c(n)) {
      case 7: need = pip_ws<7>(n); break;
      case 10: need = pip_ws<10>(n); break;
      case 11: need = pip_ws<11>(n); break;
        default: need = pip_ws<16>(n); break;
    }
  }
  int rc = ensure_ws(c, reserved + need);
  if (rc) return rc;
  char* base = static_cast<char*>(c->ws);
  if (n) {
    HIP_TRY(hipMemcpyAsync(base + o_sc, scalars, (size_t)n * 32, hipMemcpyHostToDevice, c->stream));
    HIP_TRY(hipMemcpyAsync(base + o_pts, points, (size_t)n * 32, hipMemcpyHostToDevice, c->stream));
  }
  prof_begin(c);
  rc = msm_optional_impl(c, n, reinterpret_cast<uint8_t*>(base + o_sc), reinterpret_cast<uint8_t*>(base + o_pts),
                         reinterpret_cast<uint8_t*>(base + o_out), reinterpret_cast<uint32_t*>(base + o_st), reserved);
  if (rc) return rc;
  uint32_t st = 1;
  HIP_TRY(hipMemcpyAsync(out_point, static_cast<char*>(c->ws) + o_out, 32, hipMemcpyDeviceToHost, c->stream));
  HIP_TRY(hipMemcpyAsync(&st, static_cast<char*>(c->ws) + o_st, 4, hipMemcpyDeviceToHost, c->stream));
  HIP_TRY(hipStreamSynchronize(c->stream));
  *status = (int)st;
  return ZKP_OK;
}

int zkp_decode_check(zkp_ctx* c, uint64_t n, const uint8_t* points, uint8_t* status, uint8_t* xyzt) {
  if (!c) return fail(ZKP_ERR_ARG, "ctx is NULL");
  if (n == 0) return ZKP_OK;
  if (!points || !status) return fail(ZKP_ERR_ARG, "NULL pointer");
  if (n > 0x7fffffffull) return fail(ZKP_ERR_ARG, "n too large");
  HIP_TRY(hipSetDevice(c->device));
  carve cv;
  const size_t o_pts = cv.take((size_t)n * 32);
  const size_t o_st = cv.take((size_t)n);
  const size_t o_xyzt = cv.take(xyzt ? (size_t)n * 128 : 0);
  const int rc = ensure_ws(c, cv.off);
  if (rc) return rc;
  char* base = static_cast<char*>(c->ws);
  HIP_TRY(hipMemcpyAsync(base + o_pts, points, (size_t)n * 32, hipMemcpyHostToDevice, c->stream));
  prof_begin(c);
  hipLaunchKernelGGL(k_decode_check, grid1(n, 256), dim3(256), 0, c->stream, (uint32_t)n, reinterpret_cast<uint8_t*>(base + o_pts),
                     reinterpret_cast<uint8_t*>(base + o_st), xyzt ? reinterpret_cast<uint8_t*>(base + o_xyzt) : nullptr);
  prof_mark(c, ZKP_K_DECODE);
  HIP_TRY(hipGetLastError());
  HIP_TRY(hipMemcpyAsync(status, base + o_st, (size_t)n, hipMemcpyDeviceToHost, c->stream));
  if (xyzt) HIP_TRY(hipMemcpyAsync(xyzt, base + o_xyzt, (size_t)n * 128, hipMemcpyDeviceToHost, c->stream));
  HIP_TRY(hipStreamSynchronize(c->stream));
  return ZKP_OK;
}

int zkp_from_uniform_bytes_dev(zkp_ctx* c, uint64_t n, const uint8_t* d_in, uint8_t* d_out) {
  if (!c) return fail(ZKP_ERR_ARG, "ctx is NULL");
  if (n == 0) return ZKP_OK;
// ... 386 lines not shown
    return fail(ZKP_ERR_ARG, "the shared initial transcript must not lie inside d_ts_out");
  HIP_TRY(hipSetDevice(c->device));
  prof_begin(c);
  return launch_strobe_append(c, N, shared_initial, d_ts_in, d_ts_out, lab, d_msgs, msgs_len, d_offsets);
}

int zkp_transcripts_append_message(zkp_ctx* c, uint32_t N, int shared_initial, uint8_t* ts, const char* label, const uint8_t* msgs,
                                   const uint64_t* offsets) {
  strobe_label lab;
  bool done;
  int rc = strobe_call_check(c, N, label, lab, &done);
  if (rc || done) return rc;
  if (!ts || !offsets || (offsets[N] > offsets[0] && !msgs)) return fail(ZKP_ERR_ARG, "NULL pointer");
  for (uint32_t j = 0; j < N; ++j) {
    if (offsets[j + 1] < offsets[j]) return fail(ZKP_ERR_ARG, "offsets must be non-decreasing");
    if (offsets[j + 1] - offsets[j] > 0xffffffffull) return fail(ZKP_ERR_ARG, "a message is longer than 2^32 - 1 bytes");
  }
  if (!strobe_positions_ok(ts, shared_initial ? 1 : N)) return fail(ZKP_ERR_ARG, "a transcript's position byte is 166 or more");
  const uint64_t base_off = offsets[0], total = offsets[N] - offsets[0];
  std::vector<uint64_t> rebased((size_t)N + 1);
  for (uint32_t j = 0; j <= N; ++j) rebased[j] = offsets[j] - base_off;
  HIP_TRY(hipSetDevice(c->device));
  carve cv;
  const size_t o_init = cv.take(shared_initial ? 208 : 0);
  const size_t o_ts = cv.take(208 * (size_t)N);
  const size_t o_msgs = cv.take((size_t)total);
  const size_t o_off = cv.take(((size_t)N + 1) * 8);
  rc = ensure_ws(c, cv.off);
  if (rc) return rc;
  uint8_t* base = static_cast<uint8_t*>(c->ws);
  HIP_TRY(hipMemcpyAsync(base + (shared_initial ? o_init : o_ts), ts, shared_initial ? 208 : 208 * (size_t)N, hipMemcpyHostToDevice, c->stream));
  if (total) HIP_TRY(hipMemcpyAsync(base + o_msgs, msgs + base_off, (size_t)total, hipMemcpyHostToDevice, c->stream));
  HIP_TRY(hipMemcpyAsync(base + o_off, rebased.data(), ((size_t)N + 1) * 8, hipMemcpyHostToDevice, c->stream));
  prof_begin(c);
  rc = launch_strobe_append(c, N, shared_initial, base + (shared_initial ? o_init : o_ts), base + o_ts, lab, base + o_msgs, total,
                            reinterpret_cast<const uint64_t*>(base + o_off));
  if (rc) return rc;
  HIP_TRY(hipMemcpyAsync(ts, base + o_ts, 208 * (size_t)N, hipMemcpyDeviceToHost, c->stream));
  HIP_TRY(hipStreamSynchronize(c->stream));
  return ZKP_OK;
}

int zkp_transcripts_challenge_bytes_dev(zkp_ctx* c, uint32_t N, uint8_t* d_ts, const char* label, uint32_t len, uint8_t* d_out) {
  strobe_label lab;
  bool done;
  const int rc = strobe_call_check(c, N, label, lab, &done);
  if (rc || done) return rc;
  if (!d_ts || (len && !d_out)) return fail(ZKP_ERR_ARG, "NULL device pointer");
  if (!aligned16(d_ts)) return fail(ZKP_ERR_ARG, "transcripts must be 16-byte aligned");
  HIP_TRY(hipSetDevice(c->device));
  prof_begin(c);
  return launch_strobe_challenge(c, N, d_ts, lab, len, d_out);
}

int zkp_transcripts_challenge_bytes(zkp_ctx* c, uint32_t N, uint8_t* ts, const char* label, uint32_t len, uint8_t* out) {
  strobe_label lab;
  bool done;
  int rc = strobe_call_check(c, N, label, lab, &done);
  if (rc || done) return rc;
  if (!ts || (len && !out)) return fail(ZKP_ERR_ARG, "NULL pointer");
  if (!strobe_positions_ok(ts, N)) return fail(ZKP_ERR_ARG, "a transcript's position byte is 166 or more");
  HIP_TRY(hipSetDevice(c->device));
  carve cv;
  const size_t o_ts = cv.take(208 * (size_t)N);
  const size_t o_out = cv.take((size_t)N * len);
  rc = ensure_ws(c, cv.off);
  if (rc) return rc;
  uint8_t* base = static_cast<uint8_t*>(c->ws);
  HIP_TRY(hipMemcpyAsync(base + o_ts, ts, 208 * (size_t)N, hipMemcpyHostToDevice, c->stream));
  prof_begin(c);
  rc = launch_strobe_challenge(c, N, base + o_ts, lab, len, base + o_out);
  if (rc) return rc;
  HIP_TRY(hipMemcpyAsync(ts, base + o_ts, 208 * (size_t)N, hipMemcpyDeviceToHost, c->stream));
  if (len) HIP_TRY(hipMemcpyAsync(out, base + o_out, (size_t)N * len, hipMemcpyDeviceToHost, c->stream));
  HIP_TRY(hipStreamSynchronize(c->stream));
  return ZKP_OK;
}

#ifdef ZKP_BUILD_TEST_HOOKS
int zkp_debug_last_schedule(zkp_ctx* c, char* buf, size_t cap) {
  if (!c || !buf || !cap) return fail(ZKP_ERR_ARG, "bad argument");
  static const char* const names[zkp_ctx::SCH_COUNT] = {"batch_encode", "enc_groups", "opt_pip", "pip_c", "pip_part", "status_shared", "lat_split", "grouped", "comb_min",
                                                        "ladder_interleave", "riders", "straus_lanes", "straus_wins", "tr_lanes", "tr_steps", "fuse_tt", "terms_split",
                                                        "ragged_classes", "ragged_compiled", "ragged_base", "fused_plans", "pip_merge", "pip_buckets", "no_carry", "sign_fold"};
  std::string s;
  for (int i = 0; i < zkp_ctx::SCH_COUNT; ++i)
    if (c->sched[i] >= 0) s += (s.empty() ? "" : " ") + std::string(names[i]) + "=" + std::to_string(c->sched[i]);
  const size_t n = std::min(s.size(), cap - 1);
  memcpy(buf, s.data(), n);
  buf[n] = 0;
  return (int)s.size();
}

int zkp_debug_sha512(zkp_ctx* c, uint64_t n, const uint8_t* msgs, const uint64_t* offsets, uint8_t* out) {
  return hash_from_bytes_host(c, n, msgs, offsets, out, HASH_DIGEST);
}
#endif

#ifdef ZKP_BUILD_TEST_HOOKS
int zkp_debug_quad_selftest(zkp_ctx* c, uint32_t n, const uint8_t* pairs, uint8_t* out) {
  if (!c || !pairs || !out) return fail(ZKP_ERR_ARG, "NULL pointer");
  if (n == 0) return ZKP_OK;
  HIP_TRY(hipSetDevice(c->device));
  carve cv;
  const size_t o_in = cv.take((size_t)n * 64);
  const size_t o_out = cv.take((size_t)n * 128);
  const int rc = ensure_ws(c, cv.off);
  if (rc) return rc;
  char* base = static_cast<char*>(c->ws);
  HIP_TRY(hipMemcpyAsync(base + o_in, pairs, (size_t)n * 64, hipMemcpyHostToDevice, c->stream));
  hipLaunchKernelGGL(k_debug_quad, grid1((size_t)n * 4, 256), dim3(256), 0, c->stream, n, reinterpret_cast<uint8_t*>(base + o_in), reinterpret_cast<uint8_t*>(base + o_out));
  HIP_TRY(hipGetLastError());
  HIP_TRY(hipMemcpyAsync(out, base + o_out, (size_t)n * 128, hipMemcpyDeviceToHost, c->stream));
  HIP_TRY(hipStreamSynchronize(c->stream));
  return ZKP_OK;
}
#endif

#ifdef ZKP_BUILD_TEST_HOOKS
int zkp_debug_row_selftest(zkp_ctx* c, uint32_t n, const uint8_t* pairs, uint8_t* out) {
  if (!c || !pairs || !out) return fail(ZKP_ERR_ARG, "NULL pointer");
  if (n == 0) return ZKP_OK;
  HIP_TRY(hipSetDevice(c->device));
  carve cv;
  const size_t o_in = cv.take((size_t)n * 64);
  const size_t o_out = cv.take((size_t)n * 96);
  const int rc = ensure_ws(c, cv.off);
  if (rc) return rc;
  char* base = static_cast<char*>(c->ws);
  HIP_TRY(hipMemcpyAsync(base + o_in, pairs, (size_t)n * 64, hipMemcpyHostToDevice, c->stream));
  hipLaunchKernelGGL(k_debug_row, dim3(n), dim3(64), 0, c->stream, n, reinterpret_cast<uint8_t*>(base + o_in), reinterpret_cast<uint8_t*>(base + o_out));
  HIP_TRY(hipGetLastError());
  HIP_TRY(hipMemcpyAsync(out, base + o_out, (size_t)n * 96, hipMemcpyDeviceToHost, c->stream));
  HIP_TRY(hipStreamSynchronize(c->stream));
  return ZKP_OK;
}
#endif

#ifdef ZKP_BUILD_TEST_HOOKS
int zkp_debug_wave_cycles(zkp_ctx* c, uint64_t* out, uint32_t cap) {
  if (!c || !out) return fail(ZKP_ERR_ARG, "NULL pointer");
  if (!c->wave_cycles) return fail(ZKP_ERR_ARG, "ZKP_TESTOPT_WAVE_CYCLES is off");
  HIP_TRY(hipSetDevice(c->device));
  HIP_TRY(hipStreamSynchronize(c->stream));
  const uint32_t n = std::min(cap, zkp_ctx::kWaveCyclesCap);
  HIP_TRY(hipMemcpy(out, c->wave_cycles, sizeof(uint64_t) * n, hipMemcpyDeviceToHost));
  HIP_TRY(hipMemset(c->wave_cycles, 0, sizeof(uint64_t) * zkp_ctx::kWaveCyclesCap));
  return (int)n;
}

int zkp_debug_fill_workspace(zkp_ctx* c, size_t min_bytes, uint32_t word) {
  if (!c) return fail(ZKP_ERR_ARG, "ctx is NULL");
  if (c->capturing) return fail(ZKP_ERR_ARG, "graph capture: zkp_debug_fill_workspace synchronises");
  if (c->job.kind) return fail(ZKP_ERR_ARG, "a submitted job is pending on this context: zkp_ctx_job_wait first");
  HIP_TRY(hipSetDevice(c->device));
  const int rc = ensure_ws(c, min_bytes);
  if (rc) return rc;
  if (c->ws_bytes) HIP_TRY(hipMemsetD32Async(reinterpret_cast<hipDeviceptr_t>(c->ws), (int)word, c->ws_bytes / 4, c->stream));
  if (c->ws_bytes % 4)
    HIP_TRY(hipMemsetAsync(static_cast<char*>(c->ws) + (c->ws_bytes & ~(size_t)3), (int)(word & 0xff), c->ws_bytes % 4, c->stream));
  HIP_TRY(hipStreamSynchronize(c->stream));
  if (c->side_stream) HIP_TRY(hipStreamSynchronize(c->side_stream));
  return ZKP_OK;
}
size_t zkp_debug_ws_bytes(zkp_ctx* c) { return c ? c->ws_bytes : 0; }
#endif

// ... 28 lines not shown
```

### zkp_amd/engine.py

```python
from __future__ import annotations

import ctypes
import os
from typing import Optional, Sequence, Tuple

import numpy as np

from . import cabi

_HERE = os.path.dirname(os.path.abspath(__file__))
LIB_PATH = os.path.join(_HERE, "libzkp_mi355x.so")
TESTHOOKS_LIB_PATH = os.path.join(_HERE, "libzkp_mi355x_testhooks.so")
ZKP_TESTOPT_DUMMY_LAUNCHES, ZKP_TESTOPT_GENERIC_CLASSIFIER, ZKP_TESTOPT_WAVE_CYCLES, ZKP_TESTOPT_PIP_MERGE, ZKP_TESTOPT_VOUCH_REDUCED = 1001, 1002, 1003, 1004, 1005
ZKP_OPT_CT_LOOKUP, ZKP_OPT_EACH_STRAUS, ZKP_OPT_LADDER_INTERLEAVE = 9, 10, 11
ZKP_OPT_CT_MASKED_SCANS = ZKP_OPT_CT_LOOKUP
ZKP_CT_LOOKUP_XBAR, ZKP_CT_LOOKUP_SCAN, ZKP_CT_LOOKUP_LDS = 0, 1, 2
ZKP_OPT_WS_LIMIT_BYTES, ZKP_OPT_JOB_DEFER_D2H, ZKP_OPT_SYNC_SCHEDULE, ZKP_OPT_TRANSCRIPT_STEPS, ZKP_OPT_COMB_SPLIT, ZKP_OPT_JOINT_LADDER = 12, 13, 14, 15, 16, 17

ZKP_VARTIME = 0
ZKP_CT = 1
ZKP_PT_ADD, ZKP_PT_SUB = 0, 1
ZKP_DLOG_FOUND, ZKP_DLOG_INVALID, ZKP_DLOG_NOT_FOUND = 0, 1, 2
ZKP_OPT_BATCH_ENCODE_MIN = 1
(ZKP_OPT_COMB_TEETH, ZKP_OPT_CT_SINGLE_USE_TABLES, ZKP_OPT_TRANSCRIPT_LANES, ZKP_OPT_DEV_OVERLAP, ZKP_OPT_GROUPED_COMB, ZKP_OPT_TABLES_LANE,
 ZKP_OPT_FUSE_TABLES_TRANSCRIPT) = 2, 3, 4, 5, 6, 7, 8
K_NAMES = ("decode", "terms", "reduce", "sort", "bucket", "combine", "transcript", "scalars", "tables")

EXPORTS = tuple(cabi.signatures("zkp_mi355x.h"))
TEST_HOOK_EXPORTS = tuple(cabi.signatures("zkp_mi355x.h", test_hooks=True))


class ZkpError(RuntimeError):
    pass


_lib = None
_hooks_lib = None


def load_library(test_hooks: bool = False) -> ctypes.CDLL:
    global _lib, _hooks_lib
    if test_hooks and _hooks_lib is not None:
        return _hooks_lib
    if not test_hooks and _lib is not None:
        return _lib
    path = TESTHOOKS_LIB_PATH if test_hooks else LIB_PATH
    if not os.path.exists(path):
        raise ZkpError(f"{path} is missing: run `python -c 'import __graft_entry__ as g; g.build()'` "
                       "(hipcc --offload-arch=gfx950); there is no CPU fallback")
    lib = cabi.bind(ctypes.CDLL(path), "zkp_mi355x.h", test_hooks)
    if test_hooks:
        _hooks_lib = lib
    else:
        _lib = lib
    return lib


def _check(rc: int, what: str) -> None:
    if rc != 0:
        raise ZkpError(f"{what} failed with code {rc}: {load_library().zkp_last_error().decode()}")


def _u8(a, shape_last: int) -> np.ndarray:
    if len(a) == 0:
        return np.zeros((0, shape_last), np.uint8)
    a = np.ascontiguousarray(a, dtype=np.uint8)
    if a.ndim != 2 or a.shape[1] != shape_last:
        raise ValueError(f"expected uint8 array of shape [n][{shape_last}], got {a.shape}")
    return a


def _ptr(a: Optional[np.ndarray]):
    return None if a is None else a.ctypes.data_as(ctypes.c_void_p)


def messages_csr(messages) -> Tuple[np.ndarray, np.ndarray]:
    msgs = [bytes(m) for m in messages]
    offsets = np.zeros(len(msgs) + 1, np.uint64)
    offsets[1:] = np.cumsum([len(m) for m in msgs], dtype=np.uint64)
    data = np.frombuffer(b"".join(msgs) or b"\0", np.uint8).copy()
    return data, offsets


def ragged_blocks(transcripts) -> Tuple[np.ndarray, np.ndarray]:
    lib = load_library(test_hooks=True)
    ts = _u8(transcripts, 208)
    idx = np.zeros(len(ts), np.uint32)
    cap = len(ts) + 1
    blocks = np.zeros((cap, 3), np.uint32)
    n = lib.zkp_debug_ragged_blocks(_ptr(ts), len(ts), _ptr(idx), _ptr(blocks), cap)
    if n < 0:
        _check(n, "zkp_debug_ragged_blocks")
    return idx, blocks[:n]


def _csr_args(data, offsets) -> Tuple[np.ndarray, np.ndarray]:
# ... 597 lines not shown
```

Measured before the change: 4.637 million.

## Use fewer Pippenger windows for short batch-weight scalars and folded scalars

Batch verification MSM now treats the commitment-coefficient tail as 128-bit scalars, and the long scalars as folded 252-bit values. It computes a per-point window count so digits, sort tiles and combine steps only cover the live windows. The sort kernels move to a 1D grid with a tile mapping that splits short-window and long-window regions. The tail windows are sorted over only the long prefix. Scalars that exceed their declared bit width are flagged invalid, which adds a check and ties correctness to the 128-bit random weights assumption.

Result: no change. 4.622 million (-0.3%).

```diff
diff --git a/include/zkp_mi355x.h b/include/zkp_mi355x.h
--- a/include/zkp_mi355x.h
+++ b/include/zkp_mi355x.h
@@ -264,7 +264,7 @@
 int zkp_debug_ragged_blocks(const uint8_t* transcripts, uint32_t N, uint32_t* idx, uint32_t* blocks, uint32_t cap);
 int zkp_debug_fill_workspace(zkp_ctx* ctx, size_t min_bytes, uint32_t word);
 size_t zkp_debug_ws_bytes(zkp_ctx* ctx);
-enum { ZKP_TESTOPT_DUMMY_LAUNCHES = 1001, ZKP_TESTOPT_GENERIC_CLASSIFIER = 1002, ZKP_TESTOPT_WAVE_CYCLES = 1003, ZKP_TESTOPT_PIP_MERGE = 1004, ZKP_TESTOPT_VOUCH_REDUCED = 1005 };
+enum { ZKP_TESTOPT_DUMMY_LAUNCHES = 1001, ZKP_TESTOPT_GENERIC_CLASSIFIER = 1002, ZKP_TESTOPT_WAVE_CYCLES = 1003, ZKP_TESTOPT_PIP_MERGE = 1004, ZKP_TESTOPT_VOUCH_REDUCED = 1005, ZKP_TESTOPT_PIP_SHORT_TAIL = 1006 };
 #endif
 
 #ifdef __cplusplus
diff --git a/zkp_amd/csrc/fused_flows.h b/zkp_amd/csrc/fused_flows.h
--- a/zkp_amd/csrc/fused_flows.h
+++ b/zkp_amd/csrc/fused_flows.h
@@ -1197,6 +1197,10 @@
                bool overlap = false, const std::function<int()>* late_ts = nullptr, const std::function<int()>* late_scalars = nullptr, bool late_early = false) {
   const uint32_t N = pl.N, nc = pl.s.nc, ns = pl.s.ns, ni = pl.s.ni, N_each = N / K;
   const size_t n_each = (size_t)ns + ((size_t)ni + nc) * N_each;
+  pip_seg seg;
+  seg.n_long = (uint32_t)(n_each - (size_t)nc * N_each);
+  seg.long_bits = PIP_FOLDED_BITS;
+  seg.short_bits = 128;
   const ws_view w{static_cast<char*>(c->ws)};
   uint32_t* shared = nullptr;
   if (K > 1) {
@@ -1229,7 +1233,7 @@
         if (rc) { (void)side_end(c, main, true); return rc; }
       }
       if (nc) hipLaunchKernelGGL(k_transpose_commitments, grid1((size_t)N * nc, 256), dim3(256), 0, c->stream, N, nc, d_coms, d_pts + 32 * ((size_t)ns + (size_t)ni * N));
-      rc = msm_optional_impl(c, n_each, w.u8(o.sc), d_pts, d_out, d_status, o.end, shared, 1);
+      rc = msm_optional_impl(c, n_each, w.u8(o.sc), d_pts, d_out, d_status, o.end, shared, 1, seg);
       const int rc2 = side_end(c, main, true);
       if (rc || rc2) return rc ? rc : rc2;
       if (late_ts) { rc = (*late_ts)(); if (rc) return rc; }
@@ -1251,10 +1255,9 @@
   if (split) {
     const int rc = side_join(c, true);
     if (rc) return rc;
-    return msm_optional_impl(c, n_each, w.u8(o.sc), d_pts, d_out, d_status, o.end, shared, 2);
-  }
-  if (K == 1) return msm_optional_impl(c, n_each, w.u8(o.sc), d_pts, d_out, d_status, o.end, shared);
-  pip_seg seg;
+    return msm_optional_impl(c, n_each, w.u8(o.sc), d_pts, d_out, d_status, o.end, shared, 2, seg);
+  }
+  if (K == 1) return msm_optional_impl(c, n_each, w.u8(o.sc), d_pts, d_out, d_status, o.end, shared, 3, seg);
   seg.K = K; seg.ns = ns; seg.N_each = N_each;
   switch (pick_c(n_each)) {
     case 7: return pip_run<7>(c, (uint32_t)n_each, w.u8(o.sc), d_pts, d_out, d_status, o.end, shared, seg);
diff --git a/zkp_amd/csrc/pip_recode.h b/zkp_amd/csrc/pip_recode.h
--- /dev/null
+++ b/zkp_amd/csrc/pip_recode.h
@@ -0,0 +1,76 @@
+#pragma once
+#include <stdint.h>
+#include "sc25519.h"
+
+namespace zkp {
+
+template <int C>
+struct pip_cfg {
+  static constexpr int W = (256 + C - 1) / C;
+  static constexpr int W1 = W + 1;
+  static constexpr uint32_t B = 1u << (C - 1);
+  static constexpr uint32_t B1 = B + 1;
+  static constexpr uint32_t kword(int j) {
+    uint32_t r = 0;
+    for (int w = 0; w < W; ++w) {
+      const int bit = C - 1 + C * w;
+      if (bit / 32 == j) r |= 1u << (bit % 32);
+    }
+    return r;
+  }
+};
+
+constexpr int pip_windows(int C, int bits) {
+  const int W1 = (256 + C - 1) / C + 1, n = ((bits < 256 ? bits : 256) + 1) / C + 1;
+  return n < W1 ? n : W1;
+}
+constexpr int PIP_FOLDED_BITS = 252;
+
+ZKP_HD uint32_t pip_exceeds(const uint32_t f[8], uint32_t bits) {
+  uint32_t over = 0;
+#pragma unroll
+  for (int j = 0; j < 8; ++j) {
+    const uint32_t lo = 32u * (uint32_t)j;
+    over |= bits <= lo ? f[j] : (bits < lo + 32u ? f[j] >> (bits - lo) : 0u);
+  }
+  return over ? 1u : 0u;
+}
+
+template <int C, class Emit>
+ZKP_HD void pip_digits(const uint32_t s[8], uint32_t flip, int wn, Emit&& emit) {
+  using cfg = pip_cfg<C>;
+  uint32_t e[10];
+  {
+    uint64_t c = 0;
+#pragma unroll
+    for (int j = 0; j < 9; ++j) {
+      c += (uint64_t)(j < 8 ? s[j] : 0u) + cfg::kword(j);
+      e[j] = (uint32_t)c;
+      c >>= 32;
+    }
+    e[9] = 0;
+  }
+#pragma unroll
+  for (int w = 0; w < cfg::W1; ++w) {
+    const int pos = C * w, lo = pos >> 5, sh = pos & 31;
+    uint32_t v = e[lo] >> sh;
+    if (sh + C > 32) v |= e[lo + 1] << (32 - sh);
+    v &= (1u << C) - 1u;
+    uint32_t mag, neg;
+    if (w < cfg::W) {
+      neg = (uint32_t)(v < cfg::B);
+      mag = neg ? cfg::B - v : v - cfg::B;
+    } else {
+      neg = 0;
+      mag = v;
+    }
+    if (w < wn) emit(w, mag | ((neg ^ flip) << 31));
+  }
+}
+template <int C, class Emit>
+ZKP_HD void pip_recode(uint32_t s[8], int wn, Emit&& emit) {
+  const uint32_t flip = sc_fold_sign(s);
+  pip_digits<C>(s, flip, wn, emit);
+}
+
+}
diff --git a/zkp_amd/csrc/zkp_kernels.hip b/zkp_amd/csrc/zkp_kernels.hip
--- a/zkp_amd/csrc/zkp_kernels.hip
+++ b/zkp_amd/csrc/zkp_kernels.hip
@@ -26,6 +26,7 @@
 }
 
 #include "sc25519.h"
+#include "pip_recode.h"
 #include "hot_tables.h"
 #include "quad.h"
 #include "rowfe.h"
@@ -468,25 +469,33 @@
   if (i == 0) { off[0] = 0; off[1] = n; }
 }
 
-template <int C>
-struct pip_cfg {
-  static constexpr int W = (256 + C - 1) / C;
-  static constexpr int W1 = W + 1;
-  static constexpr uint32_t B = 1u << (C - 1);
-  static constexpr uint32_t B1 = B + 1;
-  static constexpr uint32_t kword(int j) {
-    uint32_t r = 0;
-    for (int w = 0; w < W; ++w) {
-      const int bit = C - 1 + C * w;
-      if (bit / 32 == j) r |= 1u << (bit % 32);
-    }
-    return r;
-  }
-};
 
 struct pip_seg {
   uint32_t K = 1, ns = 0, N_each = 0;
+  uint32_t n_long = 0xffffffffu , long_bits = 256, short_bits = 256;
 };
+struct pip_plan {
+  uint32_t n_long, W1, Wt, Ws, long_bits, short_bits, tiles, tiles_long, blocksA;
+};
+__device__ __forceinline__ bool pip_tile_of(const pip_plan& pl, uint32_t K, uint32_t lin, bool deal8, uint32_t& g, uint32_t& w, uint32_t& t) {
+  const bool tail = lin >= pl.blocksA;
+  const uint32_t Wr = tail ? pl.Wt - pl.Ws : pl.Ws, w0 = tail ? pl.Ws : 0u, tiles = tail ? pl.tiles_long : pl.tiles, WK = K * Wr;
+  if (tail) lin -= pl.blocksA;
+  if (lin >= WK * tiles) return false;
+  const uint32_t full = (WK & ~7u) * tiles;
+  if (deal8 && lin < full) {
+    const uint32_t grp = lin / (8u * tiles), r = lin - grp * 8u * tiles;
+    w = grp * 8u + (r & 7u);
+    t = r >> 3;
+  } else {
+    w = lin / tiles;
+    t = lin - w * tiles;
+  }
+  const uint32_t b = w / Wr;
+  w = w0 + (w - b * Wr);
+  g = b * pl.W1 + w;
+  return true;
+}
 __device__ __forceinline__ void pip_seg_src(const pip_seg& seg, uint32_t b, uint32_t l, size_t& si, size_t& pi) {
   si = pi = l;
   if (seg.K > 1) {
@@ -503,15 +512,14 @@
 
 template <int C, int PHASE = 3>
 __global__ void __launch_bounds__(256, 2)
-k_pip_prepare(uint32_t n, const pip_seg seg, const uint8_t* __restrict__ scalars, const uint8_t* __restrict__ points,
+k_pip_prepare(uint32_t n, const pip_seg seg, const pip_plan pl, const uint8_t* __restrict__ scalars, const uint8_t* __restrict__ points,
               dev_niels* __restrict__ niels, uint32_t* __restrict__ digits, uint32_t* __restrict__ invalid) {
-  using cfg = pip_cfg<C>;
   const uint32_t i = blockIdx.x * blockDim.x + threadIdx.x, b = blockIdx.y;
   if (i >= n) return;
   size_t si, pi;
   pip_seg_src(seg, b, i, si, pi);
   niels += (size_t)b * n;
-  digits += (size_t)b * cfg::W1 * n;
+  digits += (size_t)b * pl.W1 * n;
   if constexpr (PHASE & 1) {
     uint32_t w[8];
     load_vec<2>(w, points + 32 * pi);
@@ -523,35 +531,11 @@
     if (!ok) atomicOr(invalid + b, 1u);
   }
   if constexpr (!(PHASE & 2)) return;
-  uint32_t s[8], e[10];
+  uint32_t s[8];
   load_vec<2>(s, scalars + 32 * si);
-  const uint32_t flip = sc_fold_sign(s);
-  {
-    uint64_t c = 0;
-#pragma unroll
-    for (int j = 0; j < 9; ++j) {
-      c += (uint64_t)(j < 8 ? s[j] : 0u) + cfg::kword(j);
-      e[j] = (uint32_t)c;
-      c >>= 32;
-    }
-    e[9] = 0;
-  }
-#pragma unroll
-  for (int w = 0; w < cfg::W1; ++w) {
-    const int pos = C * w, lo = pos >> 5, sh = pos & 31;
-    uint32_t v = e[lo] >> sh;
-    if (sh + C > 32) v |= e[lo + 1] << (32 - sh);
-    v &= (1u << C) - 1u;
-    uint32_t mag, neg;
-    if (w < cfg::W) {
-      neg = (uint32_t)(v < cfg::B);
-      mag = neg ? cfg::B - v : v - cfg::B;
-    } else {
-      neg = 0;
-      mag = v;
-    }
-    digits[(size_t)w * n + i] = mag | ((neg ^ flip) << 31);
-  }
+  const bool is_long = i < pl.n_long;
+  pip_recode<C>(s, (int)(is_long ? pl.Wt : pl.Ws), [&](int w, uint32_t word) { digits[(size_t)w * n + i] = word; });
+  if (pip_exceeds(s, is_long ? pl.long_bits : pl.short_bits)) atomicOr(invalid + b, 1u);
 }
 
 __device__ __forceinline__ uint32_t part_len(uint32_t cnt, uint32_t L) {
@@ -604,13 +588,15 @@
 
 template <int C>
 __global__ void __launch_bounds__(sort_cfg<C>::THREADS)
-k_pip_tile_hist(uint32_t n, const uint32_t* __restrict__ digits, uint32_t* __restrict__ tilehist) {
+k_pip_tile_hist(uint32_t n, uint32_t K, const pip_plan pl, const uint32_t* __restrict__ digits, uint32_t* __restrict__ tilehist) {
   using cfg = pip_cfg<C>;
   __shared__ uint32_t h[cfg::B1];
-  const uint32_t w = blockIdx.y, t = blockIdx.x, tiles = gridDim.x;
+  uint32_t w, ww, t;
+  if (!pip_tile_of(pl, K, blockIdx.x, false, w, ww, t)) return;
+  const uint32_t tiles = pl.tiles, nw = ww < pl.Ws ? n : pl.n_long;
   for (uint32_t b = threadIdx.x; b < cfg::B1; b += blockDim.x) h[b] = 0;
   __syncthreads();
-  const uint32_t lo = t * sort_cfg<C>::TILE, hi = min(n, lo + sort_cfg<C>::TILE);
+  const uint32_t lo = t * sort_cfg<C>::TILE, hi = min(nw, lo + sort_cfg<C>::TILE);
   const uint32_t* d = digits + (size_t)w * n;
   for (uint32_t i = lo + threadIdx.x; i < hi; i += blockDim.x) {
     const uint32_t mag = d[i] & 0x7fffffffu;
@@ -622,11 +608,12 @@
 }
 
 __global__ void __launch_bounds__(256)
-k_pip_tile_total(uint32_t bins, uint32_t tiles, uint32_t total, const uint32_t* __restrict__ tilehist, uint32_t* __restrict__ hist) {
+k_pip_tile_total(uint32_t bins, const pip_plan pl, uint32_t total, const uint32_t* __restrict__ tilehist, uint32_t* __restrict__ hist) {
   const uint32_t g = blockIdx.x * blockDim.x + threadIdx.x;
   if (g >= total) return;
   const uint32_t w = g / bins, b = g - w * bins;
-  const uint32_t* p = tilehist + (size_t)w * tiles * bins + b;
+  const uint32_t ww = w % pl.W1, tiles = ww < pl.Ws ? pl.tiles : (ww < pl.Wt ? pl.tiles_long : 0u);
+  const uint32_t* p = tilehist + (size_t)w * pl.tiles * bins + b;
   uint32_t sum = 0, t = 0;
   for (; t + 8 <= tiles; t += 8) {
     uint32_t v[8];
@@ -639,11 +626,12 @@
   hist[g] = sum;
 }
 __global__ void __launch_bounds__(256)
-k_pip_tile_base(uint32_t bins, uint32_t tiles, uint32_t total, const uint32_t* __restrict__ start, uint32_t* __restrict__ tilehist) {
+k_pip_tile_base(uint32_t bins, const pip_plan pl, uint32_t total, const uint32_t* __restrict__ start, uint32_t* __restrict__ tilehist) {
   const uint32_t g = blockIdx.x * blockDim.x + threadIdx.x;
   if (g >= total) return;
   const uint32_t w = g / bins, b = g - w * bins;
-  uint32_t* p = tilehist + (size_t)w * tiles * bins + b;
+  const uint32_t ww = w % pl.W1, tiles = ww < pl.Ws ? pl.tiles : (ww < pl.Wt ? pl.tiles_long : 0u);
+  uint32_t* p = tilehist + (size_t)w * pl.tiles * bins + b;
   uint32_t run = start[g], t = 0;
   for (; t + 8 <= tiles; t += 8) {
     uint32_t v[8];
@@ -661,28 +649,21 @@
 
 template <int C>
 __global__ void __launch_bounds__(sort_cfg<C>::THREADS)
-k_pip_tile_scatter(uint32_t n, const uint32_t* __restrict__ digits, const uint32_t* __restrict__ tilehist,
+k_pip_tile_scatter(uint32_t n, uint32_t K, const pip_plan pl, const uint32_t* __restrict__ digits, const uint32_t* __restrict__ tilehist,
                    uint32_t* __restrict__ sorted) {
   using cfg = pip_cfg<C>;
   __shared__ uint32_t base[cfg::B1];
-  const uint32_t tiles = gridDim.x, WK = gridDim.y, lin = blockIdx.x + blockIdx.y * tiles, full = (WK & ~7u) * tiles;
-  uint32_t w, t;
+  uint32_t w, ww, t;
 #ifdef ZKP_AB_PLAIN_SCATTER
-  if (false) {
+  if (!pip_tile_of(pl, K, blockIdx.x, false, w, ww, t)) return;
 #else
-  if (lin < full) {
+  if (!pip_tile_of(pl, K, blockIdx.x, true, w, ww, t)) return;
 #endif
-    const uint32_t grp = lin / (8u * tiles), r = lin - grp * 8u * tiles;
-    w = grp * 8u + (r & 7u);
-    t = r >> 3;
-  } else {
-    w = blockIdx.y;
-    t = blockIdx.x;
-  }
+  const uint32_t tiles = pl.tiles, nw = ww < pl.Ws ? n : pl.n_long;
   const uint32_t* in = tilehist + ((size_t)w * tiles + t) * cfg::B1;
   for (uint32_t b = threadIdx.x; b < cfg::B1; b += blockDim.x) base[b] = in[b];
   __syncthreads();
-  const uint32_t lo = t * sort_cfg<C>::TILE, hi = min(n, lo + sort_cfg<C>::TILE);
+  const uint32_t lo = t * sort_cfg<C>::TILE, hi = min(nw, lo + sort_cfg<C>::TILE);
   const uint32_t* d = digits + (size_t)w * n;
   uint32_t* out = sorted + (size_t)w * n;
   for (uint32_t i = lo + threadIdx.x; i < hi; i += blockDim.x) {
@@ -882,20 +863,20 @@
 }
 
 __global__ void __launch_bounds__(256)
-k_pip_combine(int W1, int C, uint32_t in_stride, int level, int m, int shift, const dev_ext* __restrict__ A_in, const dev_ext* __restrict__ R_in,
+k_pip_combine(int W1, int Wn , int C, uint32_t in_stride, int level, int m, int shift, const dev_ext* __restrict__ A_in, const dev_ext* __restrict__ R_in,
               dev_ext* __restrict__ T_all, const uint32_t* __restrict__ invalid, uint8_t* __restrict__ out_point, uint32_t* __restrict__ status,
               uint32_t shared_flags ) {
   const uint32_t b = blockIdx.x;
   dev_ext* T = T_all + (size_t)b * W1;
   const uint32_t g = threadIdx.x >> 2;
   const int q = (int)(threadIdx.x & 3u);
-  if (g < (uint32_t)W1) pip_reduce_quad(b * (uint32_t)W1 + g, q, 1u, in_stride, 1u, level, m, shift, A_in, R_in, T_all, nullptr);
+  if (g < (uint32_t)Wn) pip_reduce_quad(b * (uint32_t)W1 + g, q, 1u, in_stride, 1u, level, m, shift, A_in, R_in, T_all, nullptr);
   __syncthreads();
   __shared__ uint32_t Tl[64 * 36];
-  if (g < (uint32_t)W1) {
+  if (g < (uint32_t)Wn) {
     qpt t;
     q_load_ext(t, T + g, q);
-    if (g + 1 < (uint32_t)W1) {
+    if (g + 1 < (uint32_t)Wn) {
       qcached cc;
       q_to_cached(cc, t, q);
       t.c = cc.c;
@@ -908,9 +889,9 @@
     rowctx rc;
     row_init(rc);
     const uint32_t at = 9u * rc.r + (rc.live ? rc.k : 0u);
-    uint32_t acc = rc.live ? Tl[36 * (W1 - 1) + at] : 0u;
+    uint32_t acc = rc.live ? Tl[36 * (Wn - 1) + at] : 0u;
 #pragma unroll 1
-    for (int k = W1 - 2; k >= 0; --k) {
+    for (int k = Wn - 2; k >= 0; --k) {
 #pragma unroll 1
       for (int d = 0; d < C; ++d) acc = row_double(rc, acc);
       const uint32_t t = rc.live ? Tl[36 * k + at] : 0u;
@@ -1601,8 +1582,9 @@
   static constexpr uint32_t kWaveCyclesCap = 1u << 20;
   enum { SCH_BATCH_ENCODE, SCH_ENC_GROUPS, SCH_OPT_PIP, SCH_PIP_C, SCH_PIP_PART, SCH_STATUS_SHARED, SCH_LAT_SPLIT, SCH_GROUPED, SCH_COMB_MIN,
          SCH_LADDER_INTERLEAVE, SCH_RIDERS, SCH_STRAUS_LANES, SCH_STRAUS_WINS, SCH_TR_LANES, SCH_TR_STEPS, SCH_FUSE_TT, SCH_TERMS_SPLIT,
-         SCH_RAGGED_CLASSES, SCH_RAGGED_COMPILED, SCH_RAGGED_BASE, SCH_FUSED_PLANS, SCH_PIP_MERGE, SCH_PIP_BUCKETS, SCH_NO_CARRY, SCH_SIGN_FOLD, SCH_COUNT };
-  int64_t sched[SCH_COUNT] = {-1, -1, -1, -1, -1, -1, -1, -1, -1, -1, -1, -1, -1, -1, -1, -1, -1, -1, -1, -1, -1, -1, -1, -1, -1};
+         SCH_RAGGED_CLASSES, SCH_RAGGED_COMPILED, SCH_RAGGED_BASE, SCH_FUSED_PLANS, SCH_PIP_MERGE, SCH_PIP_BUCKETS, SCH_NO_CARRY, SCH_SIGN_FOLD, SCH_PIP_WINDOWS, SCH_PIP_SHORT_WINDOWS, SCH_COUNT };
+  int64_t sched[SCH_COUNT] = {-1, -1, -1, -1, -1, -1, -1, -1, -1, -1, -1, -1, -1, -1, -1, -1, -1, -1, -1, -1, -1, -1, -1, -1, -1, -1, -1};
+  uint32_t debug_pip_short_tail = 0;
   int debug_pip_merge = 0;
   bool debug_vouch_reduced = false;
 #endif
@@ -2033,6 +2015,19 @@
   const uint32_t K = seg.K;
   const size_t WK = (size_t)cfg::W1 * K;
   if (WK > 65535) return fail(ZKP_ERR_ARG, "too many batches in one call");
+  pip_plan pl;
+  pl.n_long = std::min(seg.n_long, n);
+  pl.long_bits = seg.long_bits;
+  pl.short_bits = seg.short_bits;
+  pl.W1 = (uint32_t)cfg::W1;
+  pl.Wt = (uint32_t)pip_windows(C, (int)std::min<uint32_t>(seg.long_bits, 256u));
+  pl.Ws = pl.n_long < n ? std::min(pl.Wt, (uint32_t)pip_windows(C, (int)std::min<uint32_t>(seg.short_bits, 256u))) : pl.Wt;
+  pl.tiles = pip_tiles<C>(n);
+  pl.tiles_long = pip_tiles<C>(pl.n_long);
+  pl.blocksA = (K * pl.Ws * pl.tiles + 7u) & ~7u;
+  const uint32_t sort_blocks = pl.blocksA + K * (pl.Wt - pl.Ws) * pl.tiles_long;
+  ZKP_SCHED(c, PIP_WINDOWS, pl.Wt);
+  ZKP_SCHED(c, PIP_SHORT_WINDOWS, pl.Ws);
   carve cv;
   cv.off = ws_reserved;
   char* base = static_cast<char*>(c->ws);
@@ -2045,8 +2040,7 @@
   uint32_t* start = hist + nb;
   uint32_t* cursor = start + nb;
   uint32_t* vstart = reinterpret_cast<uint32_t*>(base + cv.take(WK * (cfg::B1 + 1) * 4));
-  const uint32_t tiles = pip_tiles<C>(n);
-  uint32_t* tilehist = reinterpret_cast<uint32_t*>(base + cv.take(WK * tiles * cfg::B1 * 4));
+  uint32_t* tilehist = reinterpret_cast<uint32_t*>(base + cv.take(WK * pl.tiles * cfg::B1 * 4));
   const uint32_t L = pip_part_len(n);
   const size_t vmax = pip_vmax<C>(n);
   ZKP_SCHED(c, PIP_C, C);
@@ -2063,20 +2057,20 @@
 
   if (phases == 1) {
     if (!shared_flags) return fail(ZKP_ERR_ARG, "internal: split prepare without the caller's flag words");
-    hipLaunchKernelGGL((k_pip_prepare<C, 1>), dim3((n + 255) / 256, K), dim3(256), 0, c->stream, n, seg, d_scalars, d_points, niels, digits, invalid);
+    hipLaunchKernelGGL((k_pip_prepare<C, 1>), dim3((n + 255) / 256, K), dim3(256), 0, c->stream, n, seg, pl, d_scalars, d_points, niels, digits, invalid);
     HIP_TRY(hipGetLastError());
     return ZKP_OK;
   }
   if (!shared_flags) HIP_TRY(hipMemsetAsync(invalid, 0, (size_t)K * 4, c->stream));
   prof_note(c, ZKP_K_DECODE, "k_pip_prepare<" + std::to_string(C) + ">");
-  if (phases == 2) hipLaunchKernelGGL((k_pip_prepare<C, 2>), dim3((n + 255) / 256, K), dim3(256), 0, c->stream, n, seg, d_scalars, d_points, niels, digits, invalid);
-  else hipLaunchKernelGGL((k_pip_prepare<C, 3>), dim3((n + 255) / 256, K), dim3(256), 0, c->stream, n, seg, d_scalars, d_points, niels, digits, invalid);
+  if (phases == 2) hipLaunchKernelGGL((k_pip_prepare<C, 2>), dim3((n + 255) / 256, K), dim3(256), 0, c->stream, n, seg, pl, d_scalars, d_points, niels, digits, invalid);
+  else hipLaunchKernelGGL((k_pip_prepare<C, 3>), dim3((n + 255) / 256, K), dim3(256), 0, c->stream, n, seg, pl, d_scalars, d_points, niels, digits, invalid);
   prof_mark(c, ZKP_K_DECODE);
-  hipLaunchKernelGGL(k_pip_tile_hist<C>, dim3(tiles, (unsigned)WK), dim3(sort_cfg<C>::THREADS), 0, c->stream, n, digits, tilehist);
-  hipLaunchKernelGGL(k_pip_tile_total, grid1(nb, 256), dim3(256), 0, c->stream, cfg::B1, tiles, (uint32_t)nb, tilehist, hist);
+  hipLaunchKernelGGL(k_pip_tile_hist<C>, dim3(sort_blocks), dim3(sort_cfg<C>::THREADS), 0, c->stream, n, K, pl, digits, tilehist);
+  hipLaunchKernelGGL(k_pip_tile_total, grid1(nb, 256), dim3(256), 0, c->stream, cfg::B1, pl, (uint32_t)nb, tilehist, hist);
   hipLaunchKernelGGL(k_pip_scan, dim3((unsigned)WK), dim3(256), 0, c->stream, cfg::B1, L, hist, start, cursor, vstart);
-  hipLaunchKernelGGL(k_pip_tile_base, grid1(nb, 256), dim3(256), 0, c->stream, cfg::B1, tiles, (uint32_t)nb, start, tilehist);
-  hipLaunchKernelGGL(k_pip_tile_scatter<C>, dim3(tiles, (unsigned)WK), dim3(sort_cfg<C>::THREADS), 0, c->stream, n, digits, tilehist, sorted);
+  hipLaunchKernelGGL(k_pip_tile_base, grid1(nb, 256), dim3(256), 0, c->stream, cfg::B1, pl, (uint32_t)nb, start, tilehist);
+  hipLaunchKernelGGL(k_pip_tile_scatter<C>, dim3(sort_blocks), dim3(sort_cfg<C>::THREADS), 0, c->stream, n, K, pl, digits, tilehist, sorted);
   prof_mark(c, ZKP_K_SORT);
   hipLaunchKernelGGL(k_pip_vmap, grid1(nb, 256), dim3(256), 0, c->stream, cfg::B1, (uint32_t)nb, (uint32_t)vmax, vstart, vmap);
   hipLaunchKernelGGL(k_pip_bucket_part, dim3((unsigned)((vmax + 255) / 256), (unsigned)WK), dim3(256), 0, c->stream, n, (uint32_t)cfg::W1, cfg::B1, L, (uint32_t)vmax,
@@ -2108,7 +2102,7 @@
     dev_ext* Rout = lvlR + lvl_off;
     const uint32_t total = (uint32_t)WK * n_out;
     if (n_out == 1) {
-      hipLaunchKernelGGL(k_pip_combine, dim3(K), dim3(256), 0, c->stream, cfg::W1, C, in_stride, level, (int)m, shift, Ain, Rin, Aout, invalid, d_out, d_status, shared_flags ? 1u : 0u);
+      hipLaunchKernelGGL(k_pip_combine, dim3(K), dim3(256), 0, c->stream, cfg::W1, (int)pl.Wt, C, in_stride, level, (int)m, shift, Ain, Rin, Aout, invalid, d_out, d_status, shared_flags ? 1u : 0u);
       break;
     }
     hipLaunchKernelGGL(k_pip_reduce_lvl, grid1((size_t)total * 4, 256), dim3(256), 0, c->stream, n_out, total, in_stride, n_out, level, (int)m, shift,
@@ -2631,6 +2625,7 @@
     case ZKP_TESTOPT_GENERIC_CLASSIFIER: c->stmt_classify = value == 0; return ZKP_OK;
     case ZKP_TESTOPT_PIP_MERGE: c->debug_pip_merge = value <= 2 ? (int)value : 0; return ZKP_OK;
     case ZKP_TESTOPT_VOUCH_REDUCED: c->debug_vouch_reduced = value != 0; return ZKP_OK;
+    case ZKP_TESTOPT_PIP_SHORT_TAIL: c->debug_pip_short_tail = (uint32_t)std::min<uint64_t>(value, 0xffffffffu); return ZKP_OK;
     case ZKP_TESTOPT_DUMMY_LAUNCHES: c->debug_dummy_launches = (int)std::min<uint64_t>(value, 1000); return ZKP_OK;
     case ZKP_TESTOPT_WAVE_CYCLES: {
       HIP_TRY(hipSetDevice(c->device));
@@ -3035,8 +3030,15 @@
 }
 
 static int msm_optional_impl(zkp_ctx* c, uint64_t n, const uint8_t* d_scalars, const uint8_t* d_points,
-                             uint8_t* d_out, uint32_t* d_status, size_t reserved, uint32_t* shared_flags = nullptr, int phases = 3) {
+                             uint8_t* d_out, uint32_t* d_status, size_t reserved, uint32_t* shared_flags = nullptr, int phases = 3,
+                             pip_seg seg = pip_seg() ) {
   ZKP_SCHED(c, OPT_PIP, n > kSmallOptional);
+#ifdef ZKP_BUILD_TEST_HOOKS
+  if (c->debug_pip_short_tail && seg.n_long >= n) {
+    seg.n_long = (uint32_t)(n - std::min<uint64_t>(n, c->debug_pip_short_tail));
+    seg.short_bits = 128;
+  }
+#endif
   if (n <= kSmallOptional) {
     if (shared_flags) return fail(ZKP_ERR_ARG, "internal: shared flags with a small MSM");
     carve cv;
@@ -3064,10 +3066,10 @@
   int rc = ensure_ws(c, reserved + need);
   if (rc) return rc;
   switch (cbits) {
-    case 7: return pip_run<7>(c, (uint32_t)n, d_scalars, d_points, d_out, d_status, reserved, shared_flags, pip_seg(), phases);
-    case 10: return pip_run<10>(c, (uint32_t)n, d_scalars, d_points, d_out, d_status, reserved, shared_flags, pip_seg(), phases);
-    case 11: return pip_run<11>(c, (uint32_t)n, d_scalars, d_points, d_out, d_status, reserved, shared_flags, pip_seg(), phases);
-    default: return pip_run<16>(c, (uint32_t)n, d_scalars, d_points, d_out, d_status, reserved, shared_flags, pip_seg(), phases);
+    case 7: return pip_run<7>(c, (uint32_t)n, d_scalars, d_points, d_out, d_status, reserved, shared_flags, seg, phases);
+    case 10: return pip_run<10>(c, (uint32_t)n, d_scalars, d_points, d_out, d_status, reserved, shared_flags, seg, phases);
+    case 11: return pip_run<11>(c, (uint32_t)n, d_scalars, d_points, d_out, d_status, reserved, shared_flags, seg, phases);
+    default: return pip_run<16>(c, (uint32_t)n, d_scalars, d_points, d_out, d_status, reserved, shared_flags, seg, phases);
   }
 }
 
@@ -3620,7 +3622,7 @@
   if (!c || !buf || !cap) return fail(ZKP_ERR_ARG, "bad argument");
   static const char* const names[zkp_ctx::SCH_COUNT] = {"batch_encode", "enc_groups", "opt_pip", "pip_c", "pip_part", "status_shared", "lat_split", "grouped", "comb_min",
                                                         "ladder_interleave", "riders", "straus_lanes", "straus_wins", "tr_lanes", "tr_steps", "fuse_tt", "terms_split",
-                                                        "ragged_classes", "ragged_compiled", "ragged_base", "fused_plans", "pip_merge", "pip_buckets", "no_carry", "sign_fold"};
+                                                        "ragged_classes", "ragged_compiled", "ragged_base", "fused_plans", "pip_merge", "pip_buckets", "no_carry", "sign_fold", "pip_windows", "pip_short_windows"};
   std::string s;
   for (int i = 0; i < zkp_ctx::SCH_COUNT; ++i)
     if (c->sched[i] >= 0) s += (s.empty() ? "" : " ") + std::string(names[i]) + "=" + std::to_string(c->sched[i]);
diff --git a/zkp_amd/engine.py b/zkp_amd/engine.py
--- a/zkp_amd/engine.py
+++ b/zkp_amd/engine.py
@@ -12,6 +12,7 @@
 LIB_PATH = os.path.join(_HERE, "libzkp_mi355x.so")
 TESTHOOKS_LIB_PATH = os.path.join(_HERE, "libzkp_mi355x_testhooks.so")
 ZKP_TESTOPT_DUMMY_LAUNCHES, ZKP_TESTOPT_GENERIC_CLASSIFIER, ZKP_TESTOPT_WAVE_CYCLES, ZKP_TESTOPT_PIP_MERGE, ZKP_TESTOPT_VOUCH_REDUCED = 1001, 1002, 1003, 1004, 1005
+ZKP_TESTOPT_PIP_SHORT_TAIL = 1006
 ZKP_OPT_CT_LOOKUP, ZKP_OPT_EACH_STRAUS, ZKP_OPT_LADDER_INTERLEAVE = 9, 10, 11
 ZKP_OPT_CT_MASKED_SCANS = ZKP_OPT_CT_LOOKUP
 ZKP_CT_LOOKUP_XBAR, ZKP_CT_LOOKUP_SCAN, ZKP_CT_LOOKUP_LDS = 0, 1, 2
```
